# linnil1/KIR_graph

Measured on AMD Instinct MI355X. Metric: typed 150 bp PE reads/s (pileup+EM) per GPU; achieved HBM GB/s vs roofline, higher is better.
Workload: dtype f64

## Files before the change

include/graphkir_hip.h:

```cpp
#ifndef GRAPHKIR_HIP_H
#define GRAPHKIR_HIP_H

#include <stddef.h>
#include <stdint.h>

#ifdef __cplusplus
extern "C" {
#endif

#define GK_ABI_VERSION 1

#define GK_OK 0
#define GK_ERR_NO_DEVICE (-1)
#define GK_ERR_HIP (-2)
#define GK_ERR_ARG (-3)
#define GK_ERR_ASSERT (-4)
#define GK_ERR_CAPACITY (-5)

#define GK_MAX_CIG 14
#define GK_MAX_MM 16
#define GK_MAX_INS 6
#define GK_MAX_EVENTS 22
#define GK_CIG_M 0
#define GK_CIG_I 1
// ... 42 lines not shown
  uint8_t rsv1[16];
} gk_mate_wide;

typedef struct gk_ctx gk_ctx;
typedef struct gk_index gk_index;
typedef struct gk_tab gk_tab;
typedef struct gk_lut gk_lut;
typedef uint64_t gk_dptr;

int gk_abi_version(void);
const char* gk_last_error(void);
int gk_device_count(int* n);
int gk_ctx_create(int device, gk_ctx** out);
int gk_ctx_create_priority(int device, int urgent, gk_ctx** out);
int gk_ctx_destroy(gk_ctx* ctx);
int gk_sync(gk_ctx* ctx);
int gk_device_memory(gk_ctx* ctx, int64_t* free_bytes, int64_t* total_bytes, int64_t* pool_cached_bytes);
int gk_malloc(gk_ctx* ctx, size_t bytes, gk_dptr* out);
int gk_free(gk_ctx* ctx, gk_dptr p);
int gk_memset(gk_ctx* ctx, gk_dptr p, int value, size_t bytes);
int gk_h2d(gk_ctx* ctx, gk_dptr dst, const void* src, size_t bytes);
int gk_d2h(gk_ctx* ctx, void* dst, gk_dptr src, size_t bytes);
int gk_d2d(gk_ctx* ctx, gk_dptr dst, gk_dptr src, size_t bytes);
int gk_timer_start(gk_ctx* ctx);
int gk_timer_stop_ms(gk_ctx* ctx, float* ms);
int gk_prof_enable(gk_ctx* ctx, int on);
int gk_prof_kernel_count(void);
const char* gk_prof_kernel_name(int id);
int gk_prof_collect(gk_ctx* ctx, int64_t* launches, double* total_ms);

int gk_index_create(gk_ctx* ctx, const uint64_t* key, int32_t n_var, const int32_t* gene_vbeg,
                    int32_t n_gene, gk_index** out);
int gk_index_destroy(gk_index* idx);

typedef struct gk_tab_info {
  int64_t n_pairs;
  int64_t n_valid;
  int64_t n_ids;
  int32_t n_novel;
  int32_t err_flags;
  gk_dptr d_pair_src;
  gk_dptr d_off;
  gk_dptr d_ids;
  gk_dptr d_pair_gene;
  gk_dptr d_pair_nh;
  gk_dptr d_novel_key;
} gk_tab_info;
int gk_tabulate(gk_ctx* ctx, gk_index* idx, gk_dptr d_mates, int64_t n_pairs, gk_tab** out);
int gk_tabulate_corrected(gk_ctx* ctx, gk_index* idx, gk_dptr d_mates, int64_t n_pairs, gk_dptr d_corr,
                          gk_dptr d_gene_pos0, gk_tab** out);
int gk_tabulate_spilled(gk_ctx* ctx, gk_index* idx, gk_dptr d_mates, int64_t n_pairs, gk_dptr d_corr,
                        gk_dptr d_gene_pos0, const gk_mate_wide* wide, const int64_t* spill_pair, int64_t n_spill,
                        gk_tab** out);
int gk_tab_from_csr(gk_ctx* ctx, int32_t n_var_total, int64_t n_valid, const uint32_t* off, const uint32_t* ids,
                    const uint8_t* pair_gene, const uint8_t* pair_nh, gk_tab** out);
int gk_tab_get_info(gk_tab* tab, gk_tab_info* info);
int gk_tab_destroy(gk_tab* tab);

int gk_select_gene(gk_ctx* ctx, gk_tab* tab, int gene, int multiple, gk_dptr d_rows_out, int64_t* n_out);
int gk_select_nonempty(gk_ctx* ctx, gk_tab* tab, gk_dptr d_rows, int64_t n_rows, gk_dptr d_vflag,
                       gk_dptr d_rows_out, int64_t* n_out);

int gk_variant_count(gk_ctx* ctx, gk_tab* tab, gk_dptr d_rows, int64_t n_rows, gk_dptr d_vflag,
                     gk_dptr d_cnt);
int gk_variant_count_range(gk_ctx* ctx, gk_tab* tab, gk_dptr d_rows, int64_t n_rows, gk_dptr d_vflag,
                           gk_dptr d_cnt, int32_t vbeg, int32_t vend);
int gk_variant_correct(gk_ctx* ctx, gk_tab* tab, gk_dptr d_cnt, gk_dptr d_vflag);
int gk_variant_surviving(gk_ctx* ctx, gk_tab* tab, gk_dptr d_cnt, gk_dptr d_vflag, int64_t max_out,
                         int32_t* ord_out, uint32_t* pos_out, uint32_t* neg_out, int64_t* n_out);

int gk_variant_surviving_gene(gk_ctx* ctx, gk_tab* tab, gk_dptr d_cnt, gk_dptr d_vflag, int32_t gene, int32_t vbeg,
                              int32_t vend, int64_t max_out, int32_t* ord_out, uint32_t* pos_out, uint32_t* neg_out,
                              int64_t* n_out);
int gk_sample_prepare(gk_ctx* ctx, gk_tab* tab, int32_t multiple, gk_dptr d_vflag, gk_dptr d_cnt, gk_dptr d_rows,
                      int64_t* gene_off_out);
int gk_sample_prepare_all(gk_ctx* ctx, gk_tab* tab, int32_t multiple, gk_dptr d_vflag, gk_dptr d_cnt, gk_dptr d_rows,
                          int64_t* gene_off_out, int64_t max_out, int32_t* ord_out, uint32_t* pos_out, uint32_t* neg_out,
                          int64_t* n_out, uint64_t* novel_key_out);
int gk_sample_prepare_exon(gk_ctx* ctx, gk_tab* tab, int32_t multiple, gk_dptr d_vflag, gk_dptr d_cnt, gk_dptr d_rows,
                           int64_t* gene_off_out, int64_t max_out, int32_t* ord_out, uint32_t* pos_out, uint32_t* neg_out,
                           int64_t* n_out);

int gk_compat(gk_ctx* ctx, gk_tab* tab, gk_dptr d_rows, int64_t n_rows, gk_dptr d_vflag,
              int32_t vbeg, int32_t vend, gk_dptr d_mask, int32_t words, int32_t n_allele, int32_t keep_empty,
              gk_dptr d_probs, gk_dptr d_miss, gk_dptr d_nvar);

int gk_novel_assign(gk_ctx* ctx, gk_dptr d_probs, int64_t n_rows, int32_t n_cols, const uint32_t* col_entries,
                    int32_t n_entries, gk_dptr d_code, uint16_t* code_out, uint32_t* count_out, int32_t* first_out);
int gk_novel_confusion(gk_ctx* ctx, gk_tab* tab, gk_dptr d_rows, int64_t n_rows, gk_dptr d_code, gk_dptr d_vflag,
                       int32_t vbeg, int32_t vend, gk_dptr d_carry, const int32_t* entry_col, const int32_t* entry_slot,
                       int32_t n_entries, int32_t n_slots, uint64_t* totals_out, int64_t max_out, int32_t* slot_out,
                       int32_t* ord_out, uint32_t* count_out, uint64_t* key_out, int64_t* n_out);

int gk_lut_create(gk_ctx* ctx, int32_t log2_capacity, gk_lut** out);
int gk_lut_destroy(gk_lut* lut);
int gk_lut_collect(gk_lut* lut, gk_dptr d_vals, int64_t n);
int gk_lut_pending(gk_lut* lut, int32_t* n_total, int32_t* n_known);
int gk_lut_export(gk_lut* lut, int32_t first, int32_t count, double* keys_out);
int gk_lut_define(gk_lut* lut, int32_t first, int32_t count, const double* log_vals);
int gk_lut_apply(gk_lut* lut, gk_dptr d_in, gk_dptr d_out, int64_t n);
typedef int (*gk_log10_fn)(const double* values, int64_t n, double* out);
int gk_lut_resolve(gk_lut* lut, gk_log10_fn log10_fn, int32_t* n_new, int32_t* n_known, int32_t* n_undefined);
int gk_lut_resolve_stored(gk_lut* lut, gk_log10_fn log10_fn, int32_t* n_new, int32_t* n_known, int32_t* n_undefined);
int gk_lut_known(gk_lut* lut, int32_t* n_known);
int gk_compat_log(gk_ctx* ctx, gk_tab* tab, gk_dptr d_rows, int64_t n_rows, gk_dptr d_vflag,
                  int32_t vbeg, int32_t vend, gk_dptr d_mask, int32_t words, int32_t n_allele, int32_t keep_empty,
                  gk_lut* lut, gk_dptr d_log);

int gk_maxsum(gk_ctx* ctx, gk_dptr d_L, int64_t n_rows, int64_t ld, const int32_t* ids, int32_t n_sets,
              int32_t c_prev, const int32_t* cols, int32_t n_cols, double* out);
int gk_fraction(gk_ctx* ctx, gk_dptr d_L, int64_t n_rows, int64_t ld, const int32_t* ids,
                int32_t n_sets, int32_t c, double* frac_out);
int gk_setmax(gk_ctx* ctx, gk_dptr d_L, int64_t n_rows, int64_t ld, const int32_t* ids, int32_t n_sets,
              int32_t c, gk_dptr d_P);

int gk_compat_log_miss(gk_ctx* ctx, gk_tab* tab, gk_dptr d_rows, int64_t n_rows, gk_dptr d_vflag,
                       int32_t vbeg, int32_t vend, gk_dptr d_mask, int32_t words, int32_t n_allele,
                       int32_t keep_empty, gk_lut* lut, gk_dptr d_log, gk_dptr d_miss8, int64_t ldm, gk_dptr d_flags);
int gk_miss_colsum(gk_ctx* ctx, gk_dptr d_miss8, int64_t ldm, int32_t n_cols, gk_dptr d_msum);
int gk_compat_log_miss_cols(gk_ctx* ctx, gk_tab* tab, gk_dptr d_rows, int64_t n_rows, gk_dptr d_vflag,
                            int32_t vbeg, int32_t vend, gk_dptr d_mask, int32_t words, int32_t n_allele,
                            int32_t keep_empty, gk_lut* lut, const int32_t* table_cols, int32_t n_table_cols,
                            gk_dptr d_log, gk_dptr d_miss8, int64_t ldm, gk_dptr d_flags);
int gk_compat_log_miss_narrow(gk_ctx* ctx, gk_tab* tab, gk_dptr d_rows, int64_t n_rows, gk_dptr d_vflag,
                              int32_t vbeg, int32_t vend, gk_dptr d_mask, int32_t words, int32_t n_allele,
                              int32_t keep_empty, gk_lut* lut, const int32_t* table_cols, int32_t n_table_cols,
                              gk_dptr d_log, gk_dptr d_miss8, int64_t ldm, gk_dptr d_flags, gk_dptr d_msum);
int gk_compat_patch(gk_ctx* ctx, gk_lut* lut, gk_dptr d_log, int64_t n_rows, int32_t n_allele, gk_dptr d_miss8,
                    int64_t ldm, gk_dptr d_flags);
int gk_compat_index(gk_ctx* ctx, gk_tab* tab, gk_dptr d_rows, int64_t n_rows, gk_dptr d_vflag, int32_t vbeg,
                    int32_t vend, gk_dptr d_mask, int32_t words, int32_t n_allele, int32_t keep_empty, gk_lut* lut,
                    gk_dptr d_lidx, gk_dptr d_miss8, int64_t ldm, gk_dptr d_flags);
int gk_expand_index(gk_ctx* ctx, gk_lut* lut, gk_dptr d_lidx, int64_t ldi, int64_t n_rows, int32_t n_allele, gk_dptr d_L,
                    int64_t ld);
// ... 74 lines not shown
  int32_t n_allele;
  uint32_t stream;
} gk_boot_job;
int gk_em_bootstrap(gk_ctx* ctx, const gk_boot_job* jobs, int32_t n_jobs, int32_t n_boot, uint64_t seed,
                    int32_t iter_max, double diff_threshold,
                    double* prob_out,
                    int32_t* iters_out,
                    uint32_t* counts_out);

int gk_boot_row_counts(gk_ctx* ctx, int64_t n_rows, int32_t n_boot, int32_t boot_first, uint64_t seed, uint32_t stream,
                       gk_dptr d_W, int64_t ldw);
int gk_weighted_sums(gk_ctx* ctx, gk_dptr d_V, int64_t ld, int64_t n_rows, int32_t n_sets, gk_dptr d_W, int64_t ldw,
                     int32_t n_boot, double* out);

typedef struct gk_packer gk_packer;
int gk_packer_create(const char* const* gene_names, int32_t n_genes, const char* const* ins_strings,
                     int32_t n_ins, gk_packer** out);
int gk_packer_destroy(gk_packer* pk);
int gk_packer_feed(gk_packer* pk, const char* text, size_t n_bytes, int32_t final);
int gk_packer_counts(gk_packer* pk, int64_t* n_lines, int64_t* n_reads, int64_t* n_pairs, int64_t* n_strange,
                     int64_t* n_strings);
int gk_packer_error(gk_packer* pk, int32_t* kind, int64_t* line_index);
int gk_packer_set_output(gk_packer* pk, gk_mate* mates_out, int64_t capacity);
int gk_packer_records(gk_packer* pk, gk_mate* mates_out, int64_t* pair_lines_out);
int gk_packer_spilled(gk_packer* pk, int64_t* n_spilled_pairs);
int gk_packer_spill_records(gk_packer* pk, gk_mate_wide* wide_out, int64_t* pair_index_out);
const char* gk_packer_string(gk_packer* pk, int64_t i);

typedef struct gk_bam gk_bam;
int gk_bam_open(const char* path, int32_t name_sorted, gk_bam** out);
int gk_bam_close(gk_bam* bam);
int gk_bam_info(gk_bam* bam, int64_t* n_records, int64_t* header_bytes, int32_t* n_ref);
int gk_bam_header(gk_bam* bam, char* text_out, int64_t capacity);
int gk_bam_next(gk_bam* bam, char* text_out, int64_t capacity, int64_t* n_written);
int gk_bam_pack(gk_bam* bam, struct gk_packer* packer);
int gk_bam_write(const char* path, const char* sam_text, int64_t n_bytes, int32_t coordinate_sort);
int gk_bam_write_lines(const char* path, const char* header_text, int64_t n_header, const char* sam_text,
                       int64_t n_bytes, const int64_t* line_idx, int64_t n_lines, int32_t coordinate_sort);
int gk_json_write_reads(const char* path, const char* sam_text, int64_t n_bytes, const int64_t* pair_lines,
                        int64_t n_pairs, const int64_t* src, int64_t n_rows, const uint32_t* off,
                        const uint32_t* ids, const char* const* names, int64_t n_names,
                        const char* const* genes, int32_t n_genes, const uint8_t* gene_of, const uint8_t* nh);
int gk_bam_pileup(gk_bam* bam, const int64_t* gene_off, int32_t n_gene, uint32_t* counts_out);
int gk_bam_pileup_sites(const char* path, const int64_t* sites, int64_t n_sites, const uint64_t* name_keys,
                        const int32_t* key_group, int64_t n_keys, const int32_t* site_group, uint32_t* counts_out);
int gk_sam_name_keys(const char* sam_text, int64_t n_bytes, const int64_t* line_idx, int64_t n_lines, uint64_t* keys_out);
int gk_bam_write_lines_tagged(const char* path, const char* header_text, int64_t n_header, const char* rg_text,
                              int64_t n_rg, const char* sam_text, int64_t n_bytes, const int64_t* line_idx,
                              const int32_t* line_group, int64_t n_lines, const char* const* tags, int32_t n_tags,
                              int32_t coordinate_sort);

int gk_depth(gk_ctx* ctx, gk_tab* tab, gk_dptr d_mates, int32_t multiple, const int64_t* gene_off,
             int32_t n_gene, uint32_t* depth_out);

int gk_depth_write_tsv(const char* path, const char* const* genes, const int64_t* gene_off, int32_t n_genes,
                       const uint32_t* depth);

int gk_cn_fit(gk_ctx* ctx, const double* x, const double* density, int32_t bins, const double* bases,
              int32_t n_bases, const double* dev, int32_t n_cn, int32_t first_cn, double space,
              double* loglik_out);
int gk_cn_assign(gk_ctx* ctx, const double* x, int32_t bins, double base, const double* dev, int32_t n_cn,
                 int32_t first_cn, double space, int32_t* cn_of_bin_out);

typedef struct gk_comm gk_comm;
int gk_comm_unique_id(void* id_out, size_t capacity);
int gk_comm_create(gk_ctx* ctx, const void* id, size_t id_bytes, int32_t rank, int32_t world, gk_comm** out);
int gk_comm_destroy(gk_comm* comm);
int gk_allgather_f64(gk_comm* comm, const double* send, double* recv, int64_t n);
int gk_allreduce_max_f64(gk_comm* comm, double* inout, int64_t n);
int gk_comm_barrier(gk_comm* comm);

int gk_mates_compact(gk_ctx* ctx, gk_dptr d_mates, int64_t n_mates, gk_dptr* d_compact_out, int64_t* bytes_out);
int gk_mates_expand(gk_ctx* ctx, gk_dptr d_compact, int64_t n_mates, gk_dptr d_mates_out);
int gk_mates_compact_size(const gk_mate* mates, int64_t n_mates, int32_t n_threads, int64_t* n_words_out);
int gk_mates_compact_host(const gk_mate* mates, int64_t n_mates, int32_t n_threads, uint32_t* out, int64_t capacity_words);

int gk_host_alloc(size_t bytes, void** out);
int gk_host_free(void* p);
int gk_h2d_async(gk_ctx* ctx, gk_dptr dst, const void* src, size_t bytes);

#ifdef __cplusplus
}
#endif
#endif
```

kir_graph_amd/_lib.py:

```python
from __future__ import annotations

import ctypes as C
import threading
import os
from pathlib import Path

import numpy as np

LIB_NAME = "libgraphkir_hip.so"
_lib = None


class GkError(RuntimeError):
    """Error reported by the native library."""


class GkNoDevice(GkError):
    """No HIP device: the typing path cannot run (there is no CPU fallback)."""


_MM = np.dtype([("ref_off", "<u2"), ("base", "u1"), ("rsv", "u1")])
MATE_DTYPE = np.dtype([
    ("pos0", "<u4"), ("flag", "<u2"), ("ref", "u1"), ("nh", "u1"),
    ("nm", "u1"), ("n_cig", "u1"), ("n_mm", "u1"), ("n_ins", "u1"),
    ("cig", "<u2", (14,)), ("mm", _MM, (16,)), ("ins", "<u4", (6,)),
])
assert MATE_DTYPE.itemsize == 128

MATE_WIDE_DTYPE = np.dtype([
    ("pos0", "<u4"), ("flag", "<u2"), ("ref", "u1"), ("nh", "u1"), ("nm", "u1"), ("rsv0", "u1"),
    ("n_cig", "<u2"), ("n_mm", "<u2"), ("n_ins", "<u2"),
    ("cig", "<u4", (128,)), ("mm", "<u4", (256,)), ("ins", "<u4", (120,)), ("rsv1", "u1", (16,)),
])
assert MATE_WIDE_DTYPE.itemsize == 2048
SPILLED = 0xFF

CIG_M, CIG_I, CIG_D, CIG_S = 0, 1, 2, 4
NM_ABSENT = 255
MAX_CIG, MAX_MM, MAX_INS, MAX_EV = 14, 16, 6, 22


class GeneJob(C.Structure):
    _fields_ = [
        ("d_rows", C.c_uint64), ("n_rows", C.c_int64), ("d_mask", C.c_uint64), ("d_L", C.c_uint64),
        ("d_miss8", C.c_uint64), ("ldm", C.c_int64), ("d_msum", C.c_uint64), ("d_flags", C.c_uint64),
        ("d_lidx", C.c_uint64),
        ("vbeg", C.c_int32), ("vend", C.c_int32), ("words", C.c_int32), ("n_allele", C.c_int32),
        ("n_steps", C.c_int32), ("top_n", C.c_int32), ("bound_ok", C.c_int32), ("passes", C.c_int32),
        ("indexed", C.c_int32), ("patches", C.c_int32),
        ("table_of", C.c_int32), ("n_step_cols", C.c_int32), ("step_cols", C.c_void_p), ("step_cols_off", C.c_void_p),
        ("table_cols", C.c_void_p), ("n_table_cols", C.c_int32),
    ]


class EmJob(C.Structure):
    _fields_ = [
        ("d_rows", C.c_uint64), ("n_rows", C.c_int64), ("d_mask", C.c_uint64),
        ("vbeg", C.c_int32), ("vend", C.c_int32), ("words", C.c_int32), ("n_allele", C.c_int32),
        ("n_distinct", C.c_int32), ("iterations", C.c_int32),
    ]


class BootJob(C.Structure):
    _fields_ = [
        ("sets", C.c_void_p), ("count", C.c_void_p),
        ("n_sets", C.c_int32), ("words", C.c_int32), ("n_allele", C.c_int32), ("stream", C.c_uint32),
    ]


class TabInfo(C.Structure):
    _fields_ = [
        ("n_pairs", C.c_int64), ("n_valid", C.c_int64), ("n_ids", C.c_int64),
        ("n_novel", C.c_int32), ("err_flags", C.c_int32),
        ("d_pair_src", C.c_uint64), ("d_off", C.c_uint64), ("d_ids", C.c_uint64),
        ("d_pair_gene", C.c_uint64), ("d_pair_nh", C.c_uint64), ("d_novel_key", C.c_uint64),
    ]


def libPath() -> Path:
    return Path(__file__).resolve().parent / LIB_NAME


_SIGS = {
    "gk_abi_version": (C.c_int, []),
    "gk_last_error": (C.c_char_p, []),
    "gk_device_count": (C.c_int, [C.POINTER(C.c_int)]),
    "gk_ctx_create": (C.c_int, [C.c_int, C.POINTER(C.c_void_p)]),
    "gk_ctx_create_priority": (C.c_int, [C.c_int, C.c_int, C.POINTER(C.c_void_p)]),
    "gk_ctx_destroy": (C.c_int, [C.c_void_p]),
    "gk_sync": (C.c_int, [C.c_void_p]),
    "gk_device_memory": (C.c_int, [C.c_void_p, C.POINTER(C.c_int64), C.POINTER(C.c_int64), C.POINTER(C.c_int64)]),
    "gk_malloc": (C.c_int, [C.c_void_p, C.c_size_t, C.POINTER(C.c_uint64)]),
    "gk_free": (C.c_int, [C.c_void_p, C.c_uint64]),
    "gk_memset": (C.c_int, [C.c_void_p, C.c_uint64, C.c_int, C.c_size_t]),
    "gk_h2d": (C.c_int, [C.c_void_p, C.c_uint64, C.c_void_p, C.c_size_t]),
    "gk_d2h": (C.c_int, [C.c_void_p, C.c_void_p, C.c_uint64, C.c_size_t]),
    "gk_d2d": (C.c_int, [C.c_void_p, C.c_uint64, C.c_uint64, C.c_size_t]),
    "gk_timer_start": (C.c_int, [C.c_void_p]),
    "gk_timer_stop_ms": (C.c_int, [C.c_void_p, C.POINTER(C.c_float)]),
    "gk_prof_enable": (C.c_int, [C.c_void_p, C.c_int]),
    "gk_prof_kernel_count": (C.c_int, []),
    "gk_prof_kernel_name": (C.c_char_p, [C.c_int]),
    "gk_prof_collect": (C.c_int, [C.c_void_p, C.c_void_p, C.c_void_p]),
    "gk_index_create": (C.c_int, [C.c_void_p, C.c_void_p, C.c_int32, C.c_void_p, C.c_int32, C.POINTER(C.c_void_p)]),
    "gk_index_destroy": (C.c_int, [C.c_void_p]),
    "gk_tabulate": (C.c_int, [C.c_void_p, C.c_void_p, C.c_uint64, C.c_int64, C.POINTER(C.c_void_p)]),
    "gk_tabulate_spilled": (C.c_int, [C.c_void_p, C.c_void_p, C.c_uint64, C.c_int64, C.c_uint64, C.c_uint64,
                                     C.c_void_p, C.c_void_p, C.c_int64, C.POINTER(C.c_void_p)]),
    "gk_tabulate_corrected": (C.c_int, [C.c_void_p, C.c_void_p, C.c_uint64, C.c_int64, C.c_uint64, C.c_uint64,
                                        C.POINTER(C.c_void_p)]),
    "gk_tab_from_csr": (C.c_int, [C.c_void_p, C.c_int32, C.c_int64, C.c_void_p, C.c_void_p, C.c_void_p, C.c_void_p,
                                  C.POINTER(C.c_void_p)]),
    "gk_tab_get_info": (C.c_int, [C.c_void_p, C.POINTER(TabInfo)]),
    "gk_tab_destroy": (C.c_int, [C.c_void_p]),
    "gk_select_gene": (C.c_int, [C.c_void_p, C.c_void_p, C.c_int, C.c_int, C.c_uint64, C.POINTER(C.c_int64)]),
    "gk_select_nonempty": (C.c_int, [C.c_void_p, C.c_void_p, C.c_uint64, C.c_int64, C.c_uint64, C.c_uint64,
                                     C.POINTER(C.c_int64)]),
    "gk_variant_count": (C.c_int, [C.c_void_p, C.c_void_p, C.c_uint64, C.c_int64, C.c_uint64, C.c_uint64]),
    "gk_variant_count_range": (C.c_int, [C.c_void_p, C.c_void_p, C.c_uint64, C.c_int64, C.c_uint64, C.c_uint64,
                                         C.c_int32, C.c_int32]),
    "gk_variant_surviving": (C.c_int, [C.c_void_p, C.c_void_p, C.c_uint64, C.c_uint64, C.c_int64, C.c_void_p,
                                       C.c_void_p, C.c_void_p, C.POINTER(C.c_int64)]),
    "gk_variant_surviving_gene": (C.c_int, [C.c_void_p, C.c_void_p, C.c_uint64, C.c_uint64, C.c_int32, C.c_int32, C.c_int32,
                                            C.c_int64, C.c_void_p, C.c_void_p, C.c_void_p, C.POINTER(C.c_int64)]),
    "gk_sample_prepare": (C.c_int, [C.c_void_p, C.c_void_p, C.c_int32, C.c_uint64, C.c_uint64, C.c_uint64, C.c_void_p]),
    "gk_sample_prepare_all": (C.c_int, [C.c_void_p, C.c_void_p, C.c_int32, C.c_uint64, C.c_uint64, C.c_uint64, C.c_void_p,
                                       C.c_int64, C.c_void_p, C.c_void_p, C.c_void_p, C.POINTER(C.c_int64), C.c_void_p]),
    "gk_variant_correct": (C.c_int, [C.c_void_p, C.c_void_p, C.c_uint64, C.c_uint64]),
    "gk_compat": (C.c_int, [C.c_void_p, C.c_void_p, C.c_uint64, C.c_int64, C.c_uint64, C.c_int32, C.c_int32,
                            C.c_uint64, C.c_int32, C.c_int32, C.c_int32, C.c_uint64, C.c_uint64, C.c_uint64]),
    "gk_lut_create": (C.c_int, [C.c_void_p, C.c_int32, C.POINTER(C.c_void_p)]),
    "gk_lut_destroy": (C.c_int, [C.c_void_p]),
    "gk_lut_collect": (C.c_int, [C.c_void_p, C.c_uint64, C.c_int64]),
    "gk_lut_pending": (C.c_int, [C.c_void_p, C.POINTER(C.c_int32), C.POINTER(C.c_int32)]),
    "gk_lut_export": (C.c_int, [C.c_void_p, C.c_int32, C.c_int32, C.c_void_p]),
    "gk_lut_define": (C.c_int, [C.c_void_p, C.c_int32, C.c_int32, C.c_void_p]),
    "gk_lut_apply": (C.c_int, [C.c_void_p, C.c_uint64, C.c_uint64, C.c_int64]),
    "gk_bam_open": (C.c_int, [C.c_char_p, C.c_int32, C.POINTER(C.c_void_p)]),
    "gk_bam_close": (C.c_int, [C.c_void_p]),
    "gk_bam_info": (C.c_int, [C.c_void_p, C.POINTER(C.c_int64), C.POINTER(C.c_int64), C.POINTER(C.c_int32)]),
    "gk_bam_header": (C.c_int, [C.c_void_p, C.c_char_p, C.c_int64]),
    "gk_bam_pileup": (C.c_int, [C.c_void_p, C.c_void_p, C.c_int32, C.c_void_p]),
    "gk_bam_pileup_sites": (C.c_int, [C.c_char_p, C.c_void_p, C.c_int64, C.c_void_p, C.c_void_p, C.c_int64, C.c_void_p,
                                      C.c_void_p]),
    "gk_sam_name_keys": (C.c_int, [C.c_char_p, C.c_int64, C.c_void_p, C.c_int64, C.c_void_p]),
    "gk_bam_write_lines_tagged": (C.c_int, [C.c_char_p, C.c_char_p, C.c_int64, C.c_char_p, C.c_int64, C.c_char_p,
                                            C.c_int64, C.c_void_p, C.c_void_p, C.c_int64, C.c_void_p, C.c_int32,
                                            C.c_int32]),
    "gk_novel_assign": (C.c_int, [C.c_void_p, C.c_uint64, C.c_int64, C.c_int32, C.c_void_p, C.c_int32, C.c_uint64,
                                  C.c_void_p, C.c_void_p, C.c_void_p]),
    "gk_novel_confusion": (C.c_int, [C.c_void_p, C.c_void_p, C.c_uint64, C.c_int64, C.c_uint64, C.c_uint64, C.c_int32,
                                     C.c_int32, C.c_uint64, C.c_void_p, C.c_void_p, C.c_int32, C.c_int32, C.c_void_p,
                                     C.c_int64, C.c_void_p, C.c_void_p, C.c_void_p, C.c_void_p, C.POINTER(C.c_int64)]),
    "gk_bam_write": (C.c_int, [C.c_char_p, C.c_char_p, C.c_int64, C.c_int32]),
    "gk_bam_write_lines": (C.c_int, [C.c_char_p, C.c_char_p, C.c_int64, C.c_char_p, C.c_int64, C.c_void_p, C.c_int64,
                                     C.c_int32]),
    "gk_json_write_reads": (C.c_int, [C.c_char_p, C.c_char_p, C.c_int64, C.c_void_p, C.c_int64, C.c_void_p, C.c_int64,
                                      C.c_void_p, C.c_void_p, C.c_void_p, C.c_int64, C.c_void_p, C.c_int32,
                                      C.c_void_p, C.c_void_p]),
    "gk_bam_pack": (C.c_int, [C.c_void_p, C.c_void_p]),
    "gk_bam_next": (C.c_int, [C.c_void_p, C.c_void_p, C.c_int64, C.POINTER(C.c_int64)]),
    "gk_compat_log": (C.c_int, [C.c_void_p, C.c_void_p, C.c_uint64, C.c_int64, C.c_uint64, C.c_int32, C.c_int32,
                                C.c_uint64, C.c_int32, C.c_int32, C.c_int32, C.c_void_p, C.c_uint64]),
    "gk_maxsum": (C.c_int, [C.c_void_p, C.c_uint64, C.c_int64, C.c_int64, C.c_void_p, C.c_int32, C.c_int32,
                            C.c_void_p, C.c_int32, C.c_void_p]),
    "gk_fraction": (C.c_int, [C.c_void_p, C.c_uint64, C.c_int64, C.c_int64, C.c_void_p, C.c_int32, C.c_int32,
                              C.c_void_p]),
    "gk_setmax": (C.c_int, [C.c_void_p, C.c_uint64, C.c_int64, C.c_int64, C.c_void_p, C.c_int32, C.c_int32,
                            C.c_uint64]),
    "gk_packer_create": (C.c_int, [C.c_void_p, C.c_int32, C.c_void_p, C.c_int32, C.POINTER(C.c_void_p)]),
    "gk_packer_destroy": (C.c_int, [C.c_void_p]),
    "gk_packer_feed": (C.c_int, [C.c_void_p, C.c_char_p, C.c_size_t, C.c_int32]),
    "gk_packer_counts": (C.c_int, [C.c_void_p, C.POINTER(C.c_int64), C.POINTER(C.c_int64), C.POINTER(C.c_int64),
                                   C.POINTER(C.c_int64), C.POINTER(C.c_int64)]),
    "gk_packer_error": (C.c_int, [C.c_void_p, C.POINTER(C.c_int32), C.POINTER(C.c_int64)]),
    "gk_packer_records": (C.c_int, [C.c_void_p, C.c_void_p, C.c_void_p]),
    "gk_packer_set_output": (C.c_int, [C.c_void_p, C.c_void_p, C.c_int64]),
    "gk_packer_spilled": (C.c_int, [C.c_void_p, C.POINTER(C.c_int64)]),
    "gk_packer_spill_records": (C.c_int, [C.c_void_p, C.c_void_p, C.c_void_p]),
    "gk_packer_string": (C.c_char_p, [C.c_void_p, C.c_int64]),
    "gk_depth": (C.c_int, [C.c_void_p, C.c_void_p, C.c_uint64, C.c_int32, C.c_void_p, C.c_int32, C.c_void_p]),
    "gk_depth_write_tsv": (C.c_int, [C.c_char_p, C.c_void_p, C.c_void_p, C.c_int32, C.c_void_p]),
    "gk_cn_fit": (C.c_int, [C.c_void_p, C.c_void_p, C.c_void_p, C.c_int32, C.c_void_p, C.c_int32, C.c_void_p,
                            C.c_int32, C.c_int32, C.c_double, C.c_void_p]),
    "gk_cn_assign": (C.c_int, [C.c_void_p, C.c_void_p, C.c_int32, C.c_double, C.c_void_p, C.c_int32, C.c_int32,
                               C.c_double, C.c_void_p]),
    "gk_em_sets": (C.c_int, [C.c_void_p, C.c_void_p, C.c_uint64, C.c_int64, C.c_int32, C.c_int32, C.c_uint64,
                             C.c_int32, C.c_uint64]),
    "gk_em_distinct": (C.c_int, [C.c_void_p, C.c_uint64, C.c_int64, C.c_int32, C.c_int32, C.c_void_p, C.c_void_p,
                                 C.POINTER(C.c_int32)]),
    "gk_compat_log_miss_cols": (C.c_int, [C.c_void_p, C.c_void_p, C.c_uint64, C.c_int64, C.c_uint64, C.c_int32, C.c_int32,
                                          C.c_uint64, C.c_int32, C.c_int32, C.c_int32, C.c_void_p, C.c_void_p, C.c_int32,
                                          C.c_uint64, C.c_uint64, C.c_int64, C.c_uint64]),
    "gk_compat_log_miss_narrow": (C.c_int, [C.c_void_p, C.c_void_p, C.c_uint64, C.c_int64, C.c_uint64, C.c_int32, C.c_int32,
                                            C.c_uint64, C.c_int32, C.c_int32, C.c_int32, C.c_void_p, C.c_void_p, C.c_int32,
                                            C.c_uint64, C.c_uint64, C.c_int64, C.c_uint64, C.c_uint64]),
    "gk_compat_log_miss": (C.c_int, [C.c_void_p, C.c_void_p, C.c_uint64, C.c_int64, C.c_uint64, C.c_int32, C.c_int32,
                                     C.c_uint64, C.c_int32, C.c_int32, C.c_int32, C.c_void_p, C.c_uint64, C.c_uint64,
                                     C.c_int64, C.c_uint64]),
    "gk_miss_colsum": (C.c_int, [C.c_void_p, C.c_uint64, C.c_int64, C.c_int32, C.c_uint64]),
    "gk_compat_index": (C.c_int, [C.c_void_p, C.c_void_p, C.c_uint64, C.c_int64, C.c_uint64, C.c_int32, C.c_int32,
                                  C.c_uint64, C.c_int32, C.c_int32, C.c_int32, C.c_void_p, C.c_uint64, C.c_uint64,
                                  C.c_int64, C.c_uint64]),
    "gk_expand_index": (C.c_int, [C.c_void_p, C.c_void_p, C.c_uint64, C.c_int64, C.c_int64, C.c_int32, C.c_uint64,
                                  C.c_int64]),
    "gk_bound_step": (C.c_int, [C.c_void_p, C.c_uint64, C.c_int64, C.c_int64, C.c_uint64, C.c_void_p, C.c_int32,
                                C.c_int32, C.c_void_p, C.c_int32, C.c_void_p, C.c_int32, C.c_int32, C.c_void_p,
                                C.c_void_p, C.c_void_p]),
    "gk_setsum": (C.c_int, [C.c_void_p, C.c_uint64, C.c_int64, C.c_int64, C.c_void_p, C.c_int32, C.c_int32,
                            C.c_void_p, C.c_void_p]),
    "gk_search_run": (C.c_int, [C.c_void_p, C.c_uint64, C.c_int64, C.c_int64, C.c_int32, C.c_uint64, C.c_int64,
                                C.c_uint64, C.c_void_p, C.c_int32, C.c_int32, C.c_int32, C.c_void_p, C.c_void_p,
                                C.POINTER(C.c_void_p)]),
    "gk_sample_search": (C.c_int, [C.c_void_p, C.c_void_p, C.c_int32, C.c_void_p, C.c_uint64, C.c_void_p, C.c_void_p,
                                   C.c_int32, C.c_void_p, C.c_void_p, C.c_void_p]),
    "gk_lut_resolve": (C.c_int, [C.c_void_p, C.c_void_p, C.POINTER(C.c_int32), C.POINTER(C.c_int32),
                                 C.POINTER(C.c_int32)]),
    "gk_sample_prepare_exon": (C.c_int, [C.c_void_p, C.c_void_p, C.c_int32, C.c_uint64, C.c_uint64, C.c_uint64, C.c_void_p,
                                         C.c_int64, C.c_void_p, C.c_void_p, C.c_void_p, C.POINTER(C.c_int64)]),
    "gk_sample_em": (C.c_int, [C.c_void_p, C.c_void_p, C.c_void_p, C.c_int32, C.c_int32, C.c_double, C.c_void_p, C.c_void_p]),
    "gk_mates_compact": (C.c_int, [C.c_void_p, C.c_uint64, C.c_int64, C.POINTER(C.c_uint64), C.POINTER(C.c_int64)]),
    "gk_mates_expand": (C.c_int, [C.c_void_p, C.c_uint64, C.c_int64, C.c_uint64]),
    "gk_mates_compact_size": (C.c_int, [C.c_void_p, C.c_int64, C.c_int32, C.POINTER(C.c_int64)]),
    "gk_mates_compact_host": (C.c_int, [C.c_void_p, C.c_int64, C.c_int32, C.c_void_p, C.c_int64]),
    "gk_compat_patch": (C.c_int, [C.c_void_p, C.c_void_p, C.c_uint64, C.c_int64, C.c_int32, C.c_uint64, C.c_int64, C.c_uint64]),
    "gk_lut_resolve_stored": (C.c_int, [C.c_void_p, C.c_void_p, C.POINTER(C.c_int32), C.POINTER(C.c_int32),
                                        C.POINTER(C.c_int32)]),
    "gk_lut_known": (C.c_int, [C.c_void_p, C.POINTER(C.c_int32)]),
    "gk_search_steps": (C.c_int, [C.c_void_p, C.POINTER(C.c_int32)]),
    "gk_search_info": (C.c_int, [C.c_void_p, C.c_int32, C.POINTER(C.c_int32), C.POINTER(C.c_int64),
                                 C.POINTER(C.c_int32)]),
    "gk_search_copy": (C.c_int, [C.c_void_p, C.c_int32, C.c_void_p, C.c_void_p, C.c_void_p, C.c_void_p]),
    "gk_search_export": (C.c_int, [C.c_void_p, C.c_int32, C.c_void_p, C.c_void_p, C.c_void_p, C.c_void_p, C.c_void_p, C.c_void_p]),
    "gk_search_colsum": (C.c_int, [C.c_void_p, C.c_void_p]),
    "gk_search_log": (C.c_int, [C.c_void_p, C.c_void_p, C.c_int64, C.POINTER(C.c_int64)]),
    "gk_search_destroy": (C.c_int, [C.c_void_p]),
    "gk_site_verdict_tallies": (C.c_int, [C.c_void_p, C.c_int64, C.c_void_p, C.c_int64, C.c_void_p, C.c_void_p, C.c_void_p,
                                         C.c_int64, C.c_int32, C.POINTER(C.c_int32)]),
    "gk_site_verdict_genes": (C.c_int, [C.c_void_p, C.c_int64, C.c_void_p, C.c_int64, C.c_void_p, C.c_void_p, C.c_void_p,
                                       C.c_void_p, C.c_int32, C.c_void_p, C.c_void_p]),
    "gk_site_verdict": (C.c_int, [C.c_void_p, C.c_void_p, C.c_void_p, C.c_void_p, C.c_int64, C.c_int32,
                                  C.POINTER(C.c_int32)]),
    "gk_comm_unique_id": (C.c_int, [C.c_void_p, C.c_size_t]),
    "gk_comm_create": (C.c_int, [C.c_void_p, C.c_void_p, C.c_size_t, C.c_int32, C.c_int32, C.POINTER(C.c_void_p)]),
    "gk_comm_destroy": (C.c_int, [C.c_void_p]),
    "gk_allgather_f64": (C.c_int, [C.c_void_p, C.c_void_p, C.c_void_p, C.c_int64]),
    "gk_allreduce_max_f64": (C.c_int, [C.c_void_p, C.c_void_p, C.c_int64]),
    "gk_comm_barrier": (C.c_int, [C.c_void_p]),
    "gk_host_alloc": (C.c_int, [C.c_size_t, C.POINTER(C.c_void_p)]),
    "gk_host_free": (C.c_int, [C.c_void_p]),
    "gk_h2d_async": (C.c_int, [C.c_void_p, C.c_uint64, C.c_void_p, C.c_size_t]),
    "gk_em_run": (C.c_int, [C.c_void_p, C.c_void_p, C.c_void_p, C.c_int32, C.c_int32, C.c_int32, C.c_int32,
                            C.c_double, C.c_void_p, C.POINTER(C.c_int32)]),
    "gk_em_bootstrap": (C.c_int, [C.c_void_p, C.c_void_p, C.c_int32, C.c_int32, C.c_uint64, C.c_int32, C.c_double,
                                  C.c_void_p, C.c_void_p, C.c_void_p]),
    "gk_boot_row_counts": (C.c_int, [C.c_void_p, C.c_int64, C.c_int32, C.c_int32, C.c_uint64, C.c_uint32, C.c_uint64,
                                     C.c_int64]),
    "gk_weighted_sums": (C.c_int, [C.c_void_p, C.c_uint64, C.c_int64, C.c_int64, C.c_int32, C.c_uint64, C.c_int64, C.c_int32,
                                   C.c_void_p]),
}

EXPORTED = sorted(_SIGS)

ARGSORT_FN = C.CFUNCTYPE(C.c_int, C.POINTER(C.c_double), C.c_int64, C.POINTER(C.c_int64))


def _numpy_argsort(values, n, order_out):
    try:
        v = np.ctypeslib.as_array(values, shape=(n,))
        np.ctypeslib.as_array(order_out, shape=(n,))[:] = np.argsort(v)
        return 0
    except Exception:
# ... 249 lines not shown
```

kir_graph_amd/cohort.py:

```python
from __future__ import annotations

import os

import numpy as np


def prefetched(items, prepare, depth: int = 1, workers: int = 1):
    from concurrent.futures import ThreadPoolExecutor
    items = iter(items)
    with ThreadPoolExecutor(max_workers=max(1, workers), thread_name_prefix="gk-prefetch") as pool:
        pending = []
        for item in items:
            pending.append(pool.submit(prepare, item))
            if len(pending) > depth:
                yield pending.pop(0).result()
        while pending:
            yield pending.pop(0).result()


def overlapped(items, work, lanes: int = 2):
    from concurrent.futures import ThreadPoolExecutor
    import queue
    if lanes <= 1:
        for item in items:
# ... 29 lines not shown
        quota, period = open("/sys/fs/cgroup/cpu.max").read().split()[:2]
        if quota != "max":
            cores = min(cores, max(1, int(quota) // int(period)))
    except (OSError, ValueError):
        pass
    private = os.environ.get("GK_PRIVATE_CORES") == "1"
    ranks = 1 if private else max(1, int(os.environ.get("LOCAL_WORLD_SIZE") or os.environ.get("WORLD_SIZE") or 1))
    return max(1, cores // ranks)


def pipelineDefaults(procs: int = 1, cores: int | None = None) -> None:
    cores = hostCoresPerRank() if cores is None else cores
    lanes, slots = (5, 3) if cores >= 6 else (4, 2) if cores >= 3 else (3, 2)
    os.environ.setdefault("GK_WAIT_POLICY", "block")
    os.environ.setdefault("GK_SAMPLE_LANES", str(lanes))
    os.environ.setdefault("GK_SEARCH_SLOTS", str(slots))


def sampleLanes() -> int:
    return max(1, int(os.environ.get("GK_SAMPLE_LANES", "3")))


def stagingContexts(dev, lanes: int | None = None):
    lanes = sampleLanes() if lanes is None else lanes
    base = lanes
    ingest = dev.worker(base, urgent=True)
    return dev.worker(base + 1), ingest


def stagedSamples(items, copy_in, tabulate, depth: int | None = None):
    depth = int(os.environ.get("GK_PREFETCH", "1")) if depth is None else depth
    if depth <= 0:
        for item in items:
            yield tabulate(item if copy_in is None else copy_in(item))
        return
    if copy_in is None:
        yield from prefetched(items, tabulate, depth=depth)
    else:
        yield from prefetched(prefetched(items, copy_in, depth=depth), tabulate, depth=depth)


def sampleFootprint(data, method: str) -> int:
    tab = getattr(data, "tab", None)
    if tab is None:
        return 0
    tables = getattr(data.index, "tables", None) or []
    mean_alleles = sum(t.n_allele for t in tables) / max(len(tables), 1)
    n = int(tab.n_valid)
    if method in ("em", "report"):
        per_read = 4.0 * (mean_alleles / 32 + 1) + 16
    else:
        per_read = 9.2 * mean_alleles * (2 if method.startswith(("exonfirst", "pv_exonfirst")) else 1)
    lists = 4.0 * int(tab.n_ids) + 48.0 * n
    records = 256.0 * int(tab.n_pairs) if getattr(tab, "mates", None) is not None else 0.0
    return int(1.15 * per_read * n + lists + records)


def hbmBudget(dev=None) -> int:
    env = os.environ.get("GK_HBM_BUDGET_GB")
    if env:
        return int(float(env) * (1 << 30))
    try:
        if dev is None:
            from .kir_typing import defaultDevice
            dev = defaultDevice()
        return int(0.55 * dev.memory()[1])
    except Exception:
        return 0


class SampleTyper:

    def __init__(self, method: str, lanes: int | None = None, top_n: int = 600, variant_correction: bool = True,
                 finish=None, **typer_kwargs):
        from concurrent.futures import ThreadPoolExecutor
        import queue
        self.method = "exonfirst_1" if method == "exonfirst" else method
        self.lanes = sampleLanes() if lanes is None else max(1, lanes)
        self.top_n, self.variant_correction = top_n, variant_correction
        self.finish = finish
        self.typer_kwargs = typer_kwargs
        self._pool = ThreadPoolExecutor(max_workers=self.lanes, thread_name_prefix="gk-sample") if self.lanes > 1 else None
        self._free = queue.SimpleQueue()
        for lane in range(self.lanes):
            self._free.put(lane)
        self._pending: list = []
        import threading
        self._room = threading.Condition()
        self._inflight_bytes, self._budget = 0, None

    def _admit(self, data) -> int:
        need = sampleFootprint(data, self.method)
        if need <= 0 or self._pool is None:
            return 0
        if self._budget is None:
            self._budget = hbmBudget(getattr(getattr(data, "tab", None), "dev", None))
        if self._budget <= 0:
            return 0
        with self._room:
            while self._inflight_bytes > 0 and self._inflight_bytes + need > self._budget:
                self._room.wait(timeout=1.0)
            self._inflight_bytes += need
        return need

    def _release(self, need: int) -> None:
        if need:
            with self._room:
                self._inflight_bytes -= need
                self._room.notify_all()

    def typeOne(self, data, gene_cn, item=None, lane: int = 0):
        from .kir_typing import selectKirTypingModel
        typer = selectKirTypingModel(self.method, data, top_n=self.top_n, variant_correction=self.variant_correction,
                                     **self.typer_kwargs)
        typer.slot_base = lane
        calls, warnings = typer.typing(gene_cn() if callable(gene_cn) else gene_cn)
        if self.finish is not None:
            return self.finish(typer, calls, warnings, item)
        return calls, warnings, typer

    def _run(self, data, gene_cn, item, need: int = 0):
        lane = self._free.get()
        try:
            return self.typeOne(data, gene_cn, item, lane)
        finally:
            self._free.put(lane)
            self._release(need)

    def submit(self, data, gene_cn, item=None) -> None:
        if self._pool is None:
            self._pending.append(_Done(self.typeOne(data, gene_cn, item, 0)))
        else:
            self._pending.append(self._pool.submit(self._run, data, gene_cn, item, self._admit(data)))

    def inFlight(self) -> int:
        return len(self._pending)

    def next(self):
        return self._pending.pop(0).result()

    def drain(self):
        while self._pending:
            yield self.next()

    def close(self) -> None:
        if self._pool is not None:
            self._pool.shutdown(wait=True)
            self._pool = None

    def __enter__(self):
        return self

    def __exit__(self, *exc):
        self.close()


class _Done:
    def __init__(self, value):
        self._value = value

    def result(self):
        return self._value


def typeSamples(samples, method: str, lanes: int | None = None, finish=None, top_n: int = 600,
                variant_correction: bool = True):
    with SampleTyper(method, lanes=lanes, top_n=top_n, variant_correction=variant_correction, finish=finish) as typer:
        for data, gene_cn, item in samples:
            typer.submit(data, gene_cn, item)
            if typer.inFlight() >= typer.lanes:
                yield typer.next()
        yield from typer.drain()


def shardSamples(n_samples: int, world: int, weights=None) -> list[list[int]]:
    if weights is None:
        return [list(range(r, n_samples, world)) for r in range(world)]
    assert len(weights) == n_samples
    load = [0.0] * world
    shards: list[list[int]] = [[] for _ in range(world)]
    for i in sorted(range(n_samples), key=lambda i: (-float(weights[i]), i)):
        r = min(range(world), key=lambda r: (load[r], len(shards[r]), r))
        shards[r].append(i)
        load[r] += float(weights[i])
    return [sorted(s) for s in shards]


def sampleWeights(paths: list) -> list[float] | None:
    out = []
    for group in paths:
        total = 0
        for p in ([group] if isinstance(group, str) else group):
            if not p:
                continue
            try:
                total += os.path.getsize(p)
            except OSError:
                return None
        out.append(float(total))
    return out if any(out) else None

# ... 52 lines not shown
```

kir_graph_amd/csrc/gk_depth.hip:

```cpp
#include "gk_common.h"

namespace {

constexpr int kThreads = 256;

__global__ __launch_bounds__(kThreads) void depth_mark(const gk_mate* __restrict__ mates,
                                                       const gk_mate_wide* __restrict__ wide,
                                                       const int32_t* __restrict__ pair_src,
                                                       const uint8_t* __restrict__ pair_nh, int64_t n_valid,
                                                       int multiple, const int64_t* __restrict__ gene_off, int n_gene,
                                                       uint32_t* __restrict__ diff) {
  const int64_t t = (int64_t)blockIdx.x * kThreads + threadIdx.x;
  if (t >= 2 * n_valid) return;
  const int64_t i = t >> 1;
  if (!multiple && pair_nh[i] != 1) return;
  const gk_mate& m = mates[2 * (int64_t)pair_src[i] + (t & 1)];
  if (m.ref >= n_gene) return;
  const int64_t base = gene_off[m.ref], len = gene_off[m.ref + 1] - base;
  int64_t cur = m.pos0;
  auto run = [&](uint32_t op, uint32_t n) {
    if (op == GK_CIG_M) {
      const int64_t a = cur < 0 ? 0 : cur, b = cur + n > len ? len : cur + n;
      if (b > a) {
        atomicAdd(&diff[base + a], 1u);
        atomicAdd(&diff[base + b], 0xFFFFFFFFu);
      }
      cur += n;
    } else if (op == GK_CIG_D) {
      cur += n;
    }
  };
  if (m.n_cig == GK_SPILLED) {
    if (!wide) return;
    const gk_mate_wide& x = wide[2 * (int64_t)m.ins[0] + (t & 1)];
    const int n_cig = x.n_cig < GK_WIDE_CIG ? x.n_cig : GK_WIDE_CIG;
    for (int c = 0; c < n_cig; ++c) run(x.cig[c] & 15u, x.cig[c] >> 4);
    return;
  }
  const int n_cig = m.n_cig < GK_MAX_CIG ? m.n_cig : GK_MAX_CIG;
  for (int c = 0; c < n_cig; ++c) run(m.cig[c] & 15u, m.cig[c] >> 4);
}

__global__ __launch_bounds__(kThreads) void depth_finish(const uint32_t* excl, const uint32_t* diff, int64_t n,
                                                         uint32_t* depth ) {
  const int64_t i = (int64_t)blockIdx.x * kThreads + threadIdx.x;
  if (i < n) depth[i] = excl[i] + diff[i];
}

}

extern "C" int gk_depth(gk_ctx* ctx, gk_tab* tab, gk_dptr d_mates, int32_t multiple, const int64_t* gene_off,
                        int32_t n_gene, uint32_t* depth_out) {
  gk_bind(ctx);
  GK_REQUIRE(ctx && tab && gene_off && depth_out && n_gene > 0, "bad depth arguments");
  GK_REQUIRE(tab->d_pair_src, "depth needs a tabulation made from packed records");
  const int64_t total = gene_off[n_gene];
  hipStream_t st = ctx->stream;
  uint32_t *diff = nullptr, *scan = nullptr;
  int64_t* d_off = nullptr;
  GK_HIP(gk_pool_malloc(ctx, (void**)&diff, (size_t)(total + 1) * sizeof(uint32_t)));
  GK_HIP(gk_pool_malloc(ctx, (void**)&scan, (size_t)(total + 1) * sizeof(uint32_t)));
  GK_HIP(gk_pool_malloc(ctx, (void**)&d_off, (size_t)(n_gene + 1) * sizeof(int64_t)));
  GK_HIP(hipMemsetAsync(diff, 0, (size_t)(total + 1) * sizeof(uint32_t), st));
  GK_HIP(hipMemcpyAsync(d_off, gene_off, (size_t)(n_gene + 1) * sizeof(int64_t), hipMemcpyHostToDevice, st));
  if (tab->n_valid)
    GK_KERNEL(depth_mark, dim3((unsigned)((2 * tab->n_valid + kThreads - 1) / kThreads)), dim3(kThreads), 0, st,
                       gk_ptr<const gk_mate>(d_mates), tab->d_wide, tab->d_pair_src, tab->d_pair_nh, tab->n_valid, multiple, d_off,
                       n_gene, diff);
  GK_HIP(hipMemcpyAsync(scan, diff, (size_t)(total + 1) * sizeof(uint32_t), hipMemcpyDeviceToDevice, st));
  int rc = gk_scan_u32(ctx, scan, total + 1, nullptr);
  if (rc) return rc;
  GK_KERNEL(depth_finish, dim3((unsigned)((total + kThreads - 1) / kThreads)), dim3(kThreads), 0, st, scan, diff,
                     total, diff);
  GK_HIP(hipGetLastError());
  GK_HIP(hipMemcpyAsync(depth_out, diff, (size_t)total * sizeof(uint32_t), hipMemcpyDeviceToHost, st));
  GK_HIP(hipStreamSynchronize(st));
  gk_pool_free(ctx, diff);
  gk_pool_free(ctx, scan);
  gk_pool_free(ctx, d_off);
  return GK_OK;
}
```

kir_graph_amd/csrc/gk_tabulate.hip:

```cpp
#include <algorithm>
#include <vector>

#include "gk_common.h"

namespace {

constexpr int kThreads = 256;
constexpr int kMaxEv = GK_MAX_EVENTS;
constexpr uint64_t kEmpty = ~0ull;

constexpr int kMateWords = sizeof(gk_mate) / 4;
constexpr int kCigWord = 3;
constexpr int kMmWord = kCigWord + GK_MAX_CIG / 2;
constexpr int kInsWord = kMmWord + GK_MAX_MM;
static_assert(sizeof(gk_mate) == 128 && kInsWord + GK_MAX_INS == kMateWords, "gk_mate layout");
constexpr int kRecLd = kMateWords + 1;
constexpr int kEvLd = kMaxEv + 1;
constexpr int kMaskWords = 8;

constexpr uint32_t kEvNovel = 1u << 31;
constexpr uint32_t kEvIsN = 1u << 30;
constexpr uint32_t kEvOrdMask = (1u << 26) - 1;
constexpr uint32_t kEvSlotMask = (1u << 30) - 1;

struct MateView {
  static constexpr int kCapCig = GK_MAX_CIG, kCapMm = GK_MAX_MM, kCapIns = GK_MAX_INS, kCapEv = kMaxEv;
  const uint32_t* w;
  __device__ bool spilled() const { return n_cig() == GK_SPILLED; }
  __device__ uint32_t pos0() const { return w[0]; }
  __device__ uint32_t flag() const { return w[1] & 0xFFFFu; }
  __device__ uint32_t ref() const { return (w[1] >> 16) & 0xFFu; }
  __device__ uint32_t nm() const { return w[2] & 0xFFu; }
  __device__ uint32_t n_cig() const { return (w[2] >> 8) & 0xFFu; }
  __device__ uint32_t n_mm() const { return (w[2] >> 16) & 0xFFu; }
  __device__ uint32_t cig(int i) const {
    const uint32_t word = w[kCigWord + (i >> 1)];
    return (i & 1) ? (word >> 16) : (word & 0xFFFFu);
  }
  __device__ uint32_t mm_off(int i) const { return w[kMmWord + i] & 0xFFFFu; }
  __device__ uint32_t mm_base(int i) const { return (w[kMmWord + i] >> 16) & 0xFFu; }
  __device__ uint32_t ins(int i) const { return w[kInsWord + i]; }
  __device__ bool passes() const { return (flag() & 2u) && nm() != GK_NM_ABSENT && nm() <= 4u; }
};

constexpr int kHeadWords = 16;
constexpr int kHeadLd = kHeadWords + 1;
struct HeadView {
  static constexpr int kCapCig = GK_MAX_CIG, kCapMm = GK_MAX_MM, kCapIns = GK_MAX_INS, kCapEv = kMaxEv;
  const uint32_t* w;
  const uint32_t* g;
  __device__ uint32_t word(int i) const { return i < kHeadWords ? w[i] : g[i]; }
  __device__ bool spilled() const { return n_cig() == GK_SPILLED; }
  __device__ uint32_t pos0() const { return w[0]; }
  __device__ uint32_t flag() const { return w[1] & 0xFFFFu; }
  __device__ uint32_t ref() const { return (w[1] >> 16) & 0xFFu; }
  __device__ uint32_t nm() const { return w[2] & 0xFFu; }
  __device__ uint32_t n_cig() const { return (w[2] >> 8) & 0xFFu; }
  __device__ uint32_t n_mm() const { return (w[2] >> 16) & 0xFFu; }
  __device__ uint32_t cig(int i) const {
    const uint32_t x = w[kCigWord + (i >> 1)];
    return (i & 1) ? (x >> 16) : (x & 0xFFFFu);
  }
  __device__ uint32_t mm_off(int i) const { return word(kMmWord + i) & 0xFFFFu; }
  __device__ uint32_t mm_base(int i) const { return (word(kMmWord + i) >> 16) & 0xFFu; }
  __device__ uint32_t ins(int i) const { return g[kInsWord + i]; }
  __device__ bool passes() const { return (flag() & 2u) && nm() != GK_NM_ABSENT && nm() <= 4u; }
};
static_assert(kCigWord + GK_MAX_CIG / 2 <= kHeadWords, "the CIGAR lies in the staged head");

struct WideView {
  static constexpr int kCapCig = GK_WIDE_CIG, kCapMm = GK_WIDE_MM, kCapIns = GK_WIDE_INS, kCapEv = GK_WIDE_EVENTS;
  const gk_mate_wide* p;
  __device__ uint32_t pos0() const { return p->pos0; }
  __device__ uint32_t flag() const { return p->flag; }
  __device__ uint32_t ref() const { return p->ref; }
  __device__ uint32_t nm() const { return p->nm; }
  __device__ uint32_t n_cig() const { return p->n_cig; }
  __device__ uint32_t n_mm() const { return p->n_mm; }
  __device__ uint32_t cig(int i) const { return p->cig[i]; }
  __device__ uint32_t mm_off(int i) const { return p->mm[i] >> 8; }
  __device__ uint32_t mm_base(int i) const { return p->mm[i] & 0xFFu; }
  __device__ uint32_t ins(int i) const { return p->ins[i]; }
  __device__ bool passes() const { return (flag() & 2u) && nm() != GK_NM_ABSENT && nm() <= 4u; }
};
static_assert(sizeof(gk_mate_wide) == 2048, "gk_mate_wide layout");

__device__ inline void stage_heads(const gk_mate* mates, int64_t m0, int64_t n_mates, uint32_t* rec) {
  const int n_rec = (int)min<int64_t>(kThreads, n_mates - m0);
#pragma unroll
  for (int k = 0; k < kHeadWords / 4; ++k) {
    const int idx = threadIdx.x + kThreads * k;
    const int rcd = idx >> 2, part = idx & 3;
    if (rcd < n_rec) {
      const uint4 v = reinterpret_cast<const uint4*>(mates + m0 + rcd)[part];
      uint32_t* d = rec + rcd * kHeadLd + part * 4;
      d[0] = v.x; d[1] = v.y; d[2] = v.z; d[3] = v.w;
    }
  }
  __syncthreads();
}

__device__ inline void stage_mates(const gk_mate* mates, int64_t m0, int64_t n_mates, uint32_t* rec) {
  const uint4* src = reinterpret_cast<const uint4*>(mates + m0);
  const int n_vec = (int)min<int64_t>(kThreads, n_mates - m0) * (kMateWords / 4);
#pragma unroll
  for (int k = 0; k < kMateWords / 4; ++k) {
    const int idx = threadIdx.x + kThreads * k;
    if (idx < n_vec) {
      const uint4 v = src[idx];
      uint32_t* d = rec + (idx >> 3) * kRecLd + (idx & 7) * 4;
      d[0] = v.x; d[1] = v.y; d[2] = v.z; d[3] = v.w;
    }
  }
  __syncthreads();
}

struct IndexView {
  const uint64_t* key;
  const int32_t* bucket;
  const int32_t* gene_boff;
  int n_var, n_gene;
// ... 282 lines not shown
                                            uint32_t* more ) {
  auto keep_word = [&](uint32_t w, uint32_t word) {
    if (w == 0) first[0] = word; else if (w == 1) first[1] = word; else if (w == 2) first[2] = word;
    else if (w == 3) first[3] = word; else more[w - kMaskRegs] = word;
  };
  if (len == 0) return 0;
  if (any_n || len > 32u * kMaskWords) {
    uint32_t kept = 0, cur = 0;
    for (uint32_t c = 0; c < len; ++c) {
      const uint32_t i = lo + c;
      if (negative_kept(ix.key[i], (int)i, ix, ev, n_ev, any_n, right)) {
        ++kept;
        cur |= 1u << (c & 31u);
      }
      if ((c & 31u) == 31u || c + 1 == len) {
        if (c < 32u * kMaskWords) keep_word(c >> 5, cur);
        cur = 0;
      }
    }
    return kept;
  }
  uint32_t rel4[4];
#pragma unroll
  for (int q = 0; q < 4; ++q) rel4[q] = q < n_ev ? (ev.r[q] & ~kEvIsN) - lo : 0xFFFFFFFFu;
  const uint32_t n_words = (len + 31u) >> 5;
  uint32_t kept = 0;
  for (uint32_t w = 0; w < n_words; ++w) {
    const uint32_t left = len - 32u * w;
    uint32_t word = left >= 32u ? ~0u : ((1u << left) - 1u);
#pragma unroll
    for (int q = 0; q < 4; ++q) {
      const uint32_t rel = rel4[q] - 32u * w;
      if (rel < 32u) word &= ~(1u << rel);
    }
    for (int e = 4; e < n_ev; ++e) {
      const uint32_t rel = (ev.more[e - kEvRegs] & ~kEvIsN) - lo - 32u * w;
      if (rel < 32u) word &= ~(1u << rel);
    }
    const uint32_t first = lo + 32u * w, sh = first & 31u;
    const uint32_t a = ix.del_bits[first >> 5], b = ix.del_bits[(first >> 5) + 1];
    uint32_t dels = (sh ? (a >> sh) | (b << (32u - sh)) : a) & word;
    while (dels) {
      const int bit = __ffs(dels) - 1;
      dels &= dels - 1;
      const uint64_t k = ix.key[first + (uint32_t)bit];
      if (gk_key_pos(k) + gk_key_val(k) + 10u >= right) word &= ~(1u << bit);
    }
    kept += (uint32_t)__popc(word);
    keep_word(w, word);
  }
  return kept;
}

__global__ __launch_bounds__(kThreads) void tab_count(const gk_mate* mates, int64_t n_mates, IndexView ix,
                                                      NovelTable nt, uint32_t* cnt ,
                                                      uint32_t* valid , int* err_flags,
                                                      uint4* ev_save ,
                                                      uint32_t* ev_more ,
                                                      uint32_t* lo_save ,
                                                      uint4* mask_save ,
                                                      uint32_t* mask_more ) {
  __shared__ uint32_t rec[kThreads * kHeadLd];
  const int64_t m0 = (int64_t)blockIdx.x * kThreads;
  stage_heads(mates, m0, n_mates, rec);
  const int64_t m = m0 + threadIdx.x;
  const bool in = m < n_mates;
  const HeadView r{rec + threadIdx.x * kHeadLd, reinterpret_cast<const uint32_t*>(mates + (in ? m : 0))};
  EvRow ev{{0u, 0u, 0u, 0u}, ev_more + (in ? m : 0) * kEvMore, nt.keys};
  const bool ok = in && r.passes() && !r.spilled();
  const bool ok_other = __shfl_xor((int)ok, 1, 64) != 0;
  const bool pair_ok = ok && ok_other;
  const int64_t pair = m >> 1;
  const int side = (int)(m & 1);
  uint32_t n_pos = 0;
  Walked wk;
  wk.n = 0; wk.lo = wk.hi = 0; wk.right = 0; wk.any_n = 0;
  bool enumerate = false;
  if (pair_ok) {
    walk_mate<false>(r, ix, nt, m, ev, nullptr, 0, 0, wk);
    if (wk.overflow) atomicOr(err_flags, 2);
    if (wk.clipped) {
    } else if (wk.bad_window) {
      atomicOr(err_flags, 1);
    } else if (!wk.drop) {
      n_pos = wk.n;
      enumerate = true;
    }
  }
  uint32_t kept_bits[kMaskRegs] = {0u, 0u, 0u, 0u};
  const uint32_t n_neg = enumerate ? window_negatives(ix, ev, wk.n, wk.any_n, wk.right, (uint32_t)wk.lo,
                                                      (uint32_t)(wk.hi - wk.lo), kept_bits,
                                                      mask_more + (in ? m : 0) * (kMaskWords - kMaskRegs))
                                   : 0u;
  if (!in) return;
  cnt[4 * pair + side] = n_pos;
  cnt[4 * pair + 2 + side] = n_neg;
  if (side == 0) valid[pair] = pair_ok ? 1u : 0u;
  if (enumerate && (uint32_t)(wk.hi - wk.lo) > 32u * kMaskWords)
    atomicOr(err_flags, 4);
  ev_save[m] = make_uint4(ev.r[0], ev.r[1], ev.r[2], ev.r[3]);
  mask_save[m] = make_uint4(kept_bits[0], kept_bits[1], kept_bits[2], kept_bits[3]);
  lo_save[m] = (uint32_t)wk.lo;
}

constexpr int kExpandThreads = 128;
constexpr int kExpandWaves = kExpandThreads / 64;
constexpr uint32_t kExpandCap = 4096;

__global__ __launch_bounds__(kExpandThreads) void tab_expand(int64_t n_mates, int n_var, const uint32_t* rank,
                                                             const uint32_t* off, const uint32_t* valid,
                                                             const uint4* ev_save, const uint32_t* ev_more,
                                                             const uint32_t* lo_save, const uint4* mask_save,
                                                             const uint32_t* mask_more, uint32_t* ids) {
  __shared__ uint32_t stage[kExpandWaves][kExpandCap];
  const int lane = threadIdx.x & 63;
  const int wid = __builtin_amdgcn_readfirstlane(threadIdx.x >> 6);
  const int64_t m0 = ((int64_t)blockIdx.x * kExpandWaves + wid) * 64;
  if (m0 >= n_mates) return;
  const int64_t m = m0 + lane;
  const int64_t pair0 = m0 >> 1, pair_end = min<int64_t>((m0 + 64) >> 1, n_mates >> 1);
// ... 138 lines not shown
                                                     IndexView ix, NovelTable nt, uint32_t* cnt,
                                                     uint32_t* valid, int* err_flags, uint32_t* evw_all) {
  const int64_t t = (int64_t)blockIdx.x * 64 + threadIdx.x;
  const bool in = t < 2 * n_spill;
  const WideView r{wide + (in ? t : 0)};
  const bool ok = in && r.passes();
  const bool ok_other = __shfl_xor((int)ok, 1, 64) != 0;
  const bool pair_ok = ok && ok_other;
  if (!in) return;
  const int64_t pair = spill_pair[t >> 1];
  const int side = (int)(t & 1);
  uint32_t* evw = evw_all + t * GK_WIDE_EVENTS;
  uint32_t n_pos = 0, n_neg = 0;
  if (pair_ok) {
    Walked wk;
    EvPtr ev{evw, nullptr};
    walk_mate<false>(r, ix, nt, 2 * pair + side, ev, nullptr, 0, 0, wk);
    if (wk.overflow) atomicOr(err_flags, 2);
    if (wk.clipped) {
    } else if (wk.bad_window) {
      atomicOr(err_flags, 1);
    } else if (!wk.drop) {
      n_pos = (uint32_t)wk.n;
      for (int i = wk.lo; i < wk.hi; ++i)
        n_neg += negative_kept(ix.key[i], i, ix, EvView{evw}, wk.n, wk.any_n, wk.right) ? 1u : 0u;
    }
  }
  cnt[4 * pair + side] = n_pos;
  cnt[4 * pair + 2 + side] = n_neg;
  if (side == 0) valid[pair] = pair_ok ? 2u : 0u;
}

__global__ __launch_bounds__(64) void tab_emit_wide(const gk_mate_wide* wide, const int64_t* spill_pair, int64_t n_spill,
                                                    IndexView ix, NovelTable nt, const uint32_t* off,
                                                    const uint32_t* valid, uint32_t* ids, uint32_t* evw_all) {
  const int64_t t = (int64_t)blockIdx.x * 64 + threadIdx.x;
  if (t >= 2 * n_spill) return;
  const int64_t pair = spill_pair[t >> 1];
  const int side = (int)(t & 1);
  if (!valid[pair]) return;
  const uint32_t o_pos = off[4 * pair + side], o_pos_end = off[4 * pair + side + 1];
  const uint32_t o_neg = off[4 * pair + 2 + side], o_neg_end = off[4 * pair + 2 + side + 1];
  if (o_pos == o_pos_end && o_neg == o_neg_end) return;
  const WideView r{wide + t};
  uint32_t* evw = evw_all + t * GK_WIDE_EVENTS;
  Walked wk;
  EvPtr ev{evw, nullptr};
  walk_mate<true>(r, ix, nt, 2 * pair + side, ev, ids, o_pos, o_pos_end, wk);
  uint32_t at = o_neg;
  for (int i = wk.lo; i < wk.hi && at < o_neg_end; ++i)
    if (negative_kept(ix.key[i], i, ix, EvView{evw}, wk.n, wk.any_n, wk.right)) ids[at++] = (uint32_t)i;
}

__global__ __launch_bounds__(kThreads) void gather_pairs(const gk_mate* mates, const int32_t* pair_src, int64_t n_valid,
                                                         const uint32_t* off_in, uint32_t* off_out, uint8_t* gene,
                                                         uint8_t* nh, uint32_t total) {
  const int64_t i = (int64_t)blockIdx.x * kThreads + threadIdx.x;
  if (i > n_valid) return;
  if (i == n_valid) {
    off_out[4 * n_valid] = total;
    return;
  }
  const int64_t p = pair_src[i];
#pragma unroll
  for (int k = 0; k < 4; ++k) off_out[4 * i + k] = off_in[4 * p + k];
  const uint32_t w1 = reinterpret_cast<const uint32_t*>(mates + 2 * p)[1];
  gene[i] = (uint8_t)((w1 >> 16) & 0xFFu);
  nh[i] = (uint8_t)(w1 >> 24);
}

__device__ inline int mate_used_words(const uint32_t* w, int* n_cw, int* n_mm, int* n_ins) {
  const uint32_t h = w[2];
  const int n_cig = (int)((h >> 8) & 0xFFu);
  const bool spilled = n_cig == GK_SPILLED;
  *n_cw = spilled ? 0 : (min(n_cig, GK_MAX_CIG) + 1) / 2;
  *n_mm = spilled ? 0 : min((int)((h >> 16) & 0xFFu), GK_MAX_MM);
  *n_ins = spilled ? 1 : min((int)(h >> 24), GK_MAX_INS);
  return 3 + *n_cw + *n_mm + *n_ins;
}

__global__ __launch_bounds__(kThreads) void mates_count_words(const gk_mate* mates, int64_t n, uint32_t* cnt) {
  const int64_t m = (int64_t)blockIdx.x * kThreads + threadIdx.x;
  if (m >= n) return;
  int a, b, c;
  cnt[m] = (uint32_t)mate_used_words(reinterpret_cast<const uint32_t*>(mates + m), &a, &b, &c);
}

__global__ __launch_bounds__(kThreads) void mates_pack_words(const gk_mate* mates, int64_t n, const uint32_t* off,
                                                             uint32_t* off_out, uint32_t* words, uint32_t total) {
  const int64_t m = (int64_t)blockIdx.x * kThreads + threadIdx.x;
  if (m > n) return;
  if (m == n) { off_out[n] = total; return; }
  const uint32_t* w = reinterpret_cast<const uint32_t*>(mates + m);
  int n_cw, n_mm, n_ins;
  mate_used_words(w, &n_cw, &n_mm, &n_ins);
  uint32_t* d = words + off[m];
  off_out[m] = off[m];
  d[0] = w[0]; d[1] = w[1]; d[2] = w[2];
  d += 3;
  for (int i = 0; i < n_cw; ++i) d[i] = w[kCigWord + i];
  d += n_cw;
  for (int i = 0; i < n_mm; ++i) d[i] = w[kMmWord + i];
  d += n_mm;
  for (int i = 0; i < n_ins; ++i) d[i] = w[kInsWord + i];
}

__global__ __launch_bounds__(kThreads) void mates_unpack_words(const uint32_t* off, const uint32_t* words, int64_t n,
                                                               gk_mate* mates) {
  const int64_t m = (int64_t)blockIdx.x * kThreads + threadIdx.x;
  if (m >= n) return;
  const uint32_t* s = words + off[m];
  uint32_t rec[kMateWords];
#pragma unroll
  for (int i = 0; i < kMateWords; ++i) rec[i] = 0u;
  rec[0] = s[0]; rec[1] = s[1]; rec[2] = s[2];
  int n_cw, n_mm, n_ins;
  mate_used_words(rec, &n_cw, &n_mm, &n_ins);
  uint32_t* d = reinterpret_cast<uint32_t*>(mates + m);
  uint4* d4 = reinterpret_cast<uint4*>(d);
// ... 62 lines not shown
        for (int32_t v = ia; v < v1 && key[v] <= kb; ++v)
          if (key[v] == kb) at = v;
        snp_ord.push_back(at);
      }
    }
    lb_a.push_back(v1);
    lb_t.push_back(v1);
    for (int q = 0; q < 4; ++q) snp_ord.push_back(-1);
  }
  GK_HIP(gk_pool_malloc(ctx, (void**)&idx->d_snp_ord, snp_ord.size() * sizeof(int32_t)));
  GK_HIP(hipMemcpyAsync(idx->d_snp_ord, snp_ord.data(), snp_ord.size() * sizeof(int32_t), hipMemcpyHostToDevice, ctx->stream));
  GK_HIP(gk_pool_malloc(ctx, (void**)&idx->d_lb_a, lb_a.size() * sizeof(int32_t)));
  GK_HIP(gk_pool_malloc(ctx, (void**)&idx->d_lb_t, lb_t.size() * sizeof(int32_t)));
  GK_HIP(gk_pool_malloc(ctx, (void**)&idx->d_gene_pbase, pbase.size() * sizeof(int32_t)));
  GK_HIP(hipMemcpyAsync(idx->d_lb_a, lb_a.data(), lb_a.size() * sizeof(int32_t), hipMemcpyHostToDevice, ctx->stream));
  GK_HIP(hipMemcpyAsync(idx->d_lb_t, lb_t.data(), lb_t.size() * sizeof(int32_t), hipMemcpyHostToDevice, ctx->stream));
  GK_HIP(hipMemcpyAsync(idx->d_gene_pbase, pbase.data(), pbase.size() * sizeof(int32_t), hipMemcpyHostToDevice, ctx->stream));
  std::vector<uint32_t> del_bits((size_t)(n_var + 31) / 32 + 2, 0u);
  for (int32_t v = 0; v < n_var; ++v)
    if (gk_key_typ(key[v]) == GK_TYP_DEL) del_bits[(size_t)v >> 5] |= 1u << (v & 31);
  GK_HIP(gk_pool_malloc(ctx, (void**)&idx->d_del_bits, del_bits.size() * sizeof(uint32_t)));
  GK_HIP(hipMemcpyAsync(idx->d_del_bits, del_bits.data(), del_bits.size() * sizeof(uint32_t), hipMemcpyHostToDevice, ctx->stream));
  GK_HIP(hipStreamSynchronize(ctx->stream));
  *out = idx;
  return GK_OK;
}

int gk_index_destroy(gk_index* idx) {
  gk_bind(idx ? idx->ctx : nullptr);
  if (!idx) return GK_OK;
  gk_ctx* ctx = idx->ctx;
  gk_pool_free(ctx,idx->d_key);
  gk_pool_free(ctx,idx->d_gene_vbeg);
  gk_pool_free(ctx,idx->d_bucket);
  gk_pool_free(ctx,idx->d_gene_boff);
  gk_pool_free(ctx,idx->d_del_bits);
  gk_pool_free(ctx,idx->d_lb_a);
  gk_pool_free(ctx,idx->d_lb_t);
  gk_pool_free(ctx,idx->d_gene_pbase);
  gk_pool_free(ctx,idx->d_snp_ord);
  delete idx;
  return GK_OK;
}

int gk_tabulate(gk_ctx* ctx, gk_index* idx, gk_dptr d_mates_p, int64_t n_pairs, gk_tab** out) {
  return gk_tabulate_corrected(ctx, idx, d_mates_p, n_pairs, 0, 0, out);
}

int gk_tabulate_corrected(gk_ctx* ctx, gk_index* idx, gk_dptr d_mates_p, int64_t n_pairs, gk_dptr d_corr,
                          gk_dptr d_gene_pos0, gk_tab** out) {
  return gk_tabulate_spilled(ctx, idx, d_mates_p, n_pairs, d_corr, d_gene_pos0, nullptr, nullptr, 0, out);
}

static int tabulate_with_table(gk_ctx* ctx, gk_index* idx, gk_dptr d_mates_p, int64_t n_pairs, gk_dptr d_corr,
                               gk_dptr d_gene_pos0, const gk_mate_wide* wide, const int64_t* spill_pair,
                               int64_t n_spill, uint32_t log2cap, bool* table_too_small, gk_tab** out);

int gk_tabulate_spilled(gk_ctx* ctx, gk_index* idx, gk_dptr d_mates_p, int64_t n_pairs, gk_dptr d_corr,
                        gk_dptr d_gene_pos0, const gk_mate_wide* wide, const int64_t* spill_pair, int64_t n_spill,
                        gk_tab** out) {
  uint32_t log2cap = 16;
  while ((1ull << log2cap) < (uint64_t)(2 * std::max<int64_t>(n_pairs, 0)) && log2cap < 22) ++log2cap;
  log2cap = (uint32_t)std::min<long>(30, std::max<long>(4, gk_test_hook_value("novel_log2cap", (long)log2cap)));
  uint32_t log2max = 16;
  while ((1ull << log2max) < (uint64_t)(2 * std::max<int64_t>(n_pairs, 0)) * GK_WIDE_EVENTS * 2 && log2max < 30) ++log2max;
  for (;;) {
    bool too_small = false;
    const int rc = tabulate_with_table(ctx, idx, d_mates_p, n_pairs, d_corr, d_gene_pos0, wide, spill_pair, n_spill, log2cap,
                                       &too_small, out);
    if (!too_small) return rc;
    if (log2cap >= log2max) return rc;
    log2cap = std::min(log2cap + 3, log2max);
  }
}

static int tabulate_with_table(gk_ctx* ctx, gk_index* idx, gk_dptr d_mates_p, int64_t n_pairs, gk_dptr d_corr,
                               gk_dptr d_gene_pos0, const gk_mate_wide* wide, const int64_t* spill_pair,
                               int64_t n_spill, uint32_t log2cap, bool* table_too_small, gk_tab** out) {
  gk_bind(ctx);
  GK_REQUIRE(ctx && idx && out && n_pairs >= 0, "bad tabulate arguments");
  GK_REQUIRE(n_spill >= 0 && n_spill <= n_pairs && (n_spill == 0 || (wide && spill_pair)), "bad wide-pair arguments");
  for (int64_t k = 0; k < n_spill; ++k)
    GK_REQUIRE(spill_pair[k] >= 0 && spill_pair[k] < n_pairs && (k == 0 || spill_pair[k - 1] < spill_pair[k]),
               "wide pairs must name pairs of the sample, ascending");
  GK_REQUIRE((d_corr == 0) == (d_gene_pos0 == 0), "correction table and position offsets come together");
  GK_REQUIRE(n_pairs < (1ll << 26), "more than 2^26 pairs per call");
  const gk_mate* mates = gk_ptr<const gk_mate>(d_mates_p);
  const int64_t n_mates = 2 * n_pairs;
  hipStream_t st = ctx->stream;
  gk_tab* tab = new gk_tab();
  tab->ctx = ctx; tab->idx = idx; tab->n_pairs = n_pairs; tab->n_var = idx->n_var;

  NovelTable nt;
  const size_t cap = 1ull << log2cap;
  nt.mask = (uint32_t)(cap - 1);
  GK_HIP(gk_pool_malloc(ctx, (void**)&nt.keys, cap * sizeof(uint64_t)));
  GK_HIP(gk_pool_malloc(ctx, (void**)&nt.seq, cap * sizeof(uint64_t)));
  GK_HIP(gk_pool_malloc(ctx, (void**)&nt.rank, cap * sizeof(uint32_t)));
  GK_HIP(hipMemsetAsync(nt.keys, 0xFF, cap * sizeof(uint64_t), st));
  GK_HIP(hipMemsetAsync(nt.seq, 0xFF, cap * sizeof(uint64_t), st));

  uint32_t *cnt = nullptr, *valid = nullptr, *lo_save = nullptr, *ev_more = nullptr, *mask_more = nullptr;
  uint4 *ev_save = nullptr, *mask_save = nullptr;
  int* d_err = nullptr;
  GK_HIP(gk_pool_malloc(ctx, (void**)&ev_save, (size_t)(n_mates + 1) * sizeof(uint4)));
  GK_HIP(gk_pool_malloc(ctx, (void**)&ev_more, (size_t)(n_mates + 1) * kEvMore * sizeof(uint32_t)));
  GK_HIP(gk_pool_malloc(ctx, (void**)&lo_save, (size_t)(n_mates + 1) * sizeof(uint32_t)));
  GK_HIP(gk_pool_malloc(ctx, (void**)&mask_save, (size_t)(n_mates + 1) * sizeof(uint4)));
  GK_HIP(gk_pool_malloc(ctx, (void**)&mask_more, (size_t)(n_mates + 1) * (kMaskWords - kMaskRegs) * sizeof(uint32_t)));
  GK_HIP(gk_pool_malloc(ctx, (void**)&cnt, (size_t)(4 * n_pairs + 2) * sizeof(uint32_t)));
  GK_HIP(gk_pool_malloc(ctx, (void**)&valid, (size_t)(n_pairs + 1) * sizeof(uint32_t)));
  GK_HIP(gk_pool_malloc(ctx, (void**)&d_err, sizeof(int)));
  GK_HIP(hipMemsetAsync(d_err, 0, sizeof(int), st));
  nt.flags = d_err;

  const IndexView ix{idx->d_key, idx->d_bucket, idx->d_gene_boff, idx->n_var, idx->n_gene,
                     gk_ptr<uint8_t>(d_corr), gk_ptr<int64_t>(d_gene_pos0), idx->d_del_bits, idx->d_lb_a, idx->d_lb_t,
                     idx->d_gene_pbase, idx->d_snp_ord};
  if (n_mates) {
    GK_PROF(ctx, "tab_count", GK_KERNEL(tab_count, dim3(nblk(n_mates)), dim3(kThreads), 0, st, mates, n_mates, ix,
                       nt, cnt, valid, d_err, ev_save, ev_more, lo_save, mask_save, mask_more));
  }
  int64_t* d_spill_pair = nullptr;
  uint32_t* wide_ev = nullptr;
  if (n_spill) {
    GK_HIP(gk_pool_malloc(ctx, (void**)&tab->d_wide, (size_t)(2 * n_spill) * sizeof(gk_mate_wide)));
    GK_HIP(gk_pool_malloc(ctx, (void**)&d_spill_pair, (size_t)n_spill * sizeof(int64_t)));
    GK_HIP(gk_pool_malloc(ctx, (void**)&wide_ev, (size_t)(2 * n_spill) * GK_WIDE_EVENTS * sizeof(uint32_t)));
    GK_HIP(hipMemcpyAsync(tab->d_wide, wide, (size_t)(2 * n_spill) * sizeof(gk_mate_wide), hipMemcpyHostToDevice, st));
    GK_HIP(hipMemcpyAsync(d_spill_pair, spill_pair, (size_t)n_spill * sizeof(int64_t), hipMemcpyHostToDevice, st));
    GK_HIP(hipStreamSynchronize(st));
    tab->n_spill = n_spill;
    GK_KERNEL(tab_count_wide, dim3(nblk(2 * n_spill, 64)), dim3(64), 0, st, tab->d_wide, d_spill_pair, n_spill, ix, nt,
              cnt, valid, d_err, wide_ev);
  }
  int rc = gk_scan_u32(ctx, cnt, 4 * n_pairs, cnt + 4 * n_pairs);
  if (rc) return rc;

  const int64_t n_words = n_mates + 1;
  uint32_t *bitmap = nullptr, *prefix = nullptr, *wide_bits = nullptr;
  GK_HIP(gk_pool_malloc(ctx, (void**)&bitmap, (size_t)n_words * sizeof(uint32_t)));
  GK_HIP(gk_pool_malloc(ctx, (void**)&prefix, (size_t)(n_words + 1) * sizeof(uint32_t)));
  GK_HIP(gk_pool_malloc(ctx, (void**)&wide_bits, (size_t)(2 * n_spill + 1) * kWideWords * sizeof(uint32_t)));
  GK_HIP(hipMemsetAsync(bitmap, 0, (size_t)n_words * sizeof(uint32_t), st));
  GK_HIP(hipMemsetAsync(wide_bits, 0, (size_t)(2 * n_spill + 1) * kWideWords * sizeof(uint32_t), st));
  GK_PROF(ctx, "novel_mark", GK_KERNEL(novel_mark, dim3(nblk((int64_t)cap)), dim3(kThreads), 0, st, nt, bitmap, wide_bits,
                                     d_spill_pair, n_spill));
  GK_PROF(ctx, "novel_count", GK_KERNEL(novel_count, dim3(nblk(n_words)), dim3(kThreads), 0, st, bitmap, prefix, n_words));
  if (n_spill)
    GK_KERNEL(novel_count_wide, dim3(nblk(2 * n_spill)), dim3(kThreads), 0, st, wide_bits, d_spill_pair, n_spill, prefix);
  rc = gk_scan_u32(ctx, prefix, n_words, prefix + n_words);
  if (rc) return rc;

  uint32_t totals[2] = {0, 0};
  int err = 0;
  GK_HIP(gk_fetch_queue(ctx, &totals[0], cnt + 4 * n_pairs, sizeof(uint32_t)));
  GK_HIP(gk_fetch_queue(ctx, &totals[1], prefix + n_words, sizeof(uint32_t)));
  GK_HIP(gk_fetch_queue(ctx, &err, d_err, sizeof(int)));
  GK_HIP(gk_fetch_wait(ctx));
  tab->n_ids = totals[0];
  tab->n_novel = (int32_t)totals[1];
  tab->err_flags = err & 3;
  if ((err & 8) || (uint64_t)tab->n_novel * 2 > cap) {
    gk_set_error("novel variant table overflow (%d novel variants in %llu slots)", tab->n_novel, (unsigned long long)cap);
    *table_too_small = true;
    GK_HIP(hipStreamSynchronize(st));
    gk_pool_free(ctx,cnt); gk_pool_free(ctx,valid); gk_pool_free(ctx,d_err); gk_pool_free(ctx,bitmap); gk_pool_free(ctx,prefix); gk_pool_free(ctx,wide_bits);
    gk_pool_free(ctx,ev_save); gk_pool_free(ctx,lo_save); gk_pool_free(ctx,mask_save); gk_pool_free(ctx,ev_more); gk_pool_free(ctx,mask_more);
    gk_pool_free(ctx,d_spill_pair); gk_pool_free(ctx,wide_ev);
    gk_pool_free(ctx,nt.keys); gk_pool_free(ctx,nt.seq); gk_pool_free(ctx,nt.rank);
    gk_tab_destroy(tab);
    return GK_ERR_CAPACITY;
  }

  GK_HIP(gk_pool_malloc(ctx, (void**)&tab->d_novel_key, (size_t)(tab->n_novel + 1) * sizeof(uint64_t)));
  GK_PROF(ctx, "novel_assign", GK_KERNEL(novel_assign, dim3(nblk((int64_t)cap)), dim3(kThreads), 0, st, nt, bitmap, wide_bits,
                     d_spill_pair, n_spill, prefix, tab->d_novel_key));

  GK_HIP(gk_pool_malloc(ctx, (void**)&tab->d_ids, (size_t)(tab->n_ids + 1) * sizeof(uint32_t)));
  if (n_mates) {
    const bool two_walks = gk_test_hook("two_walks");
    if ((err & 4) || two_walks) {
      GK_PROF(ctx, "tab_emit", GK_KERNEL(tab_emit, dim3(nblk(n_mates)), dim3(kThreads), 0, st, mates, n_mates, ix, nt,
                         cnt, valid, tab->d_ids));
    } else {
      GK_PROF(ctx, "tab_expand", GK_KERNEL(tab_expand, dim3(nblk(n_mates, kExpandThreads)), dim3(kExpandThreads), 0, st, n_mates, idx->n_var,
                         nt.rank, cnt, valid, ev_save, ev_more, lo_save, mask_save, mask_more, tab->d_ids));
    }
    if (n_spill)
      GK_KERNEL(tab_emit_wide, dim3(nblk(2 * n_spill, 64)), dim3(64), 0, st, tab->d_wide, d_spill_pair, n_spill, ix, nt,
                cnt, valid, tab->d_ids, wide_ev);
  }
  GK_HIP(gk_pool_malloc(ctx, (void**)&tab->d_pair_src, (size_t)(n_pairs + 1) * sizeof(int32_t)));
  rc = gk_compact(ctx, valid, nullptr, n_pairs, tab->d_pair_src, &tab->n_valid);
  if (rc) return rc;
  GK_HIP(gk_pool_malloc(ctx, (void**)&tab->d_off, (size_t)(4 * tab->n_valid + 1) * sizeof(uint32_t)));
  GK_HIP(gk_pool_malloc(ctx, (void**)&tab->d_pair_gene, (size_t)tab->n_valid + 1));
  GK_HIP(gk_pool_malloc(ctx, (void**)&tab->d_pair_nh, (size_t)tab->n_valid + 1));
  GK_PROF(ctx, "gather_pairs", GK_KERNEL(gather_pairs, dim3(nblk(tab->n_valid + 1)), dim3(kThreads), 0, st, mates, tab->d_pair_src,
                     tab->n_valid, cnt, tab->d_off, tab->d_pair_gene, tab->d_pair_nh, (uint32_t)tab->n_ids));
  GK_HIP(hipGetLastError());
  GK_HIP(hipStreamSynchronize(st));
  gk_pool_free(ctx,cnt); gk_pool_free(ctx,valid); gk_pool_free(ctx,d_err); gk_pool_free(ctx,bitmap); gk_pool_free(ctx,prefix); gk_pool_free(ctx,wide_bits);
  gk_pool_free(ctx,ev_save); gk_pool_free(ctx,lo_save); gk_pool_free(ctx,mask_save); gk_pool_free(ctx,ev_more); gk_pool_free(ctx,mask_more);
  gk_pool_free(ctx,d_spill_pair); gk_pool_free(ctx,wide_ev);
  gk_pool_free(ctx,nt.keys); gk_pool_free(ctx,nt.seq); gk_pool_free(ctx,nt.rank);
  if (err & 2) {
    gk_set_error("a filter-passing mate carries more variant events than its record format allows (%d, wide %d)", kMaxEv,
                 GK_WIDE_EVENTS);
    gk_tab_destroy(tab);
    return GK_ERR_CAPACITY;
  }
  *out = tab;
  return GK_OK;
}

int gk_tab_from_csr(gk_ctx* ctx, int32_t n_var_total, int64_t n_valid, const uint32_t* off, const uint32_t* ids,
                    const uint8_t* pair_gene, const uint8_t* pair_nh, gk_tab** out) {
  gk_bind(ctx);
  GK_REQUIRE(ctx && out && off && pair_gene && pair_nh && n_valid >= 0 && n_var_total >= 0, "bad CSR arguments");
  const int64_t n_ids = off[4 * n_valid];
  for (int64_t i = 0; i < 4 * n_valid; ++i) GK_REQUIRE(off[i] <= off[i + 1], "CSR offsets must be non-decreasing");
  for (int64_t i = 0; i < n_ids; ++i) GK_REQUIRE(ids[i] < (uint32_t)n_var_total, "variant ordinal out of range");
  gk_tab* tab = new gk_tab();
  tab->ctx = ctx; tab->n_pairs = n_valid; tab->n_valid = n_valid; tab->n_ids = n_ids;
  tab->n_var = n_var_total; tab->n_novel = 0;
  hipStream_t st = ctx->stream;
  GK_HIP(gk_pool_malloc(ctx, (void**)&tab->d_off, (size_t)(4 * n_valid + 1) * sizeof(uint32_t)));
  GK_HIP(gk_pool_malloc(ctx, (void**)&tab->d_ids, (size_t)(n_ids + 1) * sizeof(uint32_t)));
  GK_HIP(gk_pool_malloc(ctx, (void**)&tab->d_pair_gene, (size_t)n_valid + 1));
  GK_HIP(gk_pool_malloc(ctx, (void**)&tab->d_pair_nh, (size_t)n_valid + 1));
  GK_HIP(hipMemcpyAsync(tab->d_off, off, (size_t)(4 * n_valid + 1) * sizeof(uint32_t), hipMemcpyHostToDevice, st));
  if (n_ids) GK_HIP(hipMemcpyAsync(tab->d_ids, ids, (size_t)n_ids * sizeof(uint32_t), hipMemcpyHostToDevice, st));
  if (n_valid) {
    GK_HIP(hipMemcpyAsync(tab->d_pair_gene, pair_gene, (size_t)n_valid, hipMemcpyHostToDevice, st));
    GK_HIP(hipMemcpyAsync(tab->d_pair_nh, pair_nh, (size_t)n_valid, hipMemcpyHostToDevice, st));
  }
  GK_HIP(hipStreamSynchronize(st));
  *out = tab;
  return GK_OK;
}

int gk_tab_get_info(gk_tab* tab, gk_tab_info* info) {
  gk_bind(tab ? tab->ctx : nullptr);
  GK_REQUIRE(tab && info, "null pointer");
  info->n_pairs = tab->n_pairs; info->n_valid = tab->n_valid; info->n_ids = tab->n_ids;
  info->n_novel = tab->n_novel; info->err_flags = tab->err_flags;
  info->d_pair_src = gk_addr(tab->d_pair_src); info->d_off = gk_addr(tab->d_off); info->d_ids = gk_addr(tab->d_ids);
  info->d_pair_gene = gk_addr(tab->d_pair_gene); info->d_pair_nh = gk_addr(tab->d_pair_nh);
  info->d_novel_key = gk_addr(tab->d_novel_key);
  return GK_OK;
}

int gk_tab_destroy(gk_tab* tab) {
  gk_bind(tab ? tab->ctx : nullptr);
  if (!tab) return GK_OK;
  gk_ctx* ctx = tab->ctx;
  gk_pool_free(ctx,tab->d_pair_src); gk_pool_free(ctx,tab->d_off); gk_pool_free(ctx,tab->d_ids);
// ... 49 lines not shown
```

kir_graph_amd/csrc/gk_typing.hip:

```cpp
#include <algorithm>

#include "gk_common.h"
#include "gk_lut.h"

namespace {

constexpr int kThreads = 256;
inline unsigned nblk(int64_t n, int t = kThreads) { return (unsigned)((n + t - 1) / t); }

template <bool kScatter>
__global__ __launch_bounds__(kThreads) void part_pass(const uint8_t* gene, const uint8_t* nh, int64_t n, int multiple,
                                                      int n_bins, int64_t n_tiles, uint32_t* hist, int32_t* out) {
  const int64_t i = (int64_t)blockIdx.x * kThreads + threadIdx.x;
  const int lane = threadIdx.x & 63;
  const int64_t tile = i >> 6;
  int bin = -1;
  if (i < n && (multiple || nh[i] == 1)) {
    bin = gene[i];
    if (bin >= n_bins) bin = -1;
  }
  uint64_t todo = __ballot(bin >= 0);
  while (todo) {
    const int leader = __ffsll((unsigned long long)todo) - 1;
    const int b = __shfl(bin, leader, 64);
// ... 8 lines not shown
}

__global__ void part_offsets(const uint32_t* hist, const uint32_t* total, int n_bins, int64_t n_tiles, uint32_t* goff) {
  const int b = blockIdx.x * blockDim.x + threadIdx.x;
  if (b < n_bins) goff[b] = hist[(int64_t)b * n_tiles];
  if (b == n_bins) goff[b] = *total;
}

__global__ __launch_bounds__(kThreads) void count_ids(const int32_t* __restrict__ rows, int64_t n_rows,
                                                      const uint32_t* __restrict__ off,
                                                      const uint32_t* __restrict__ ids,
                                                      const uint8_t* __restrict__ vflag, uint32_t* cnt_pos,
                                                      uint32_t* cnt_neg, int vbeg, int n_local) {
  extern __shared__ uint32_t hist[];
  for (int i = threadIdx.x; i < 2 * n_local; i += kThreads) hist[i] = 0;
  __syncthreads();
  constexpr int kGroup = 16;
  const int lane = threadIdx.x & (kGroup - 1);
  const int64_t group = ((int64_t)blockIdx.x * kThreads + threadIdx.x) / kGroup;
  const int64_t n_groups = ((int64_t)gridDim.x * kThreads) / kGroup;
  for (int64_t i = group; i < n_rows; i += n_groups) {
    const int64_t row = rows[i];
    const uint32_t b = off[4 * row], mid = off[4 * row + 2], e = off[4 * row + 4];
    for (uint32_t k = b + lane; k < e; k += kGroup) {
      const uint32_t v = ids[k];
      const bool positive = k < mid;
      if (vflag[v] & (positive ? 1 : 2)) continue;
      const uint32_t l = v - (uint32_t)vbeg;
      if (l < (uint32_t)n_local) atomicAdd(&hist[(positive ? 0 : n_local) + l], 1u);
      else atomicAdd(positive ? &cnt_pos[v] : &cnt_neg[v], 1u);
    }
  }
  __syncthreads();
  for (int i = threadIdx.x; i < 2 * n_local; i += kThreads) {
    const uint32_t c = hist[i];
    if (c) atomicAdd(i < n_local ? &cnt_pos[vbeg + i] : &cnt_neg[vbeg + i - n_local], c);
  }
}

__global__ __launch_bounds__(kThreads) void apply_correction(const uint32_t* cnt_pos, const uint32_t* cnt_neg,
                                                             int64_t n, uint8_t* vflag) {
  const int64_t v = (int64_t)blockIdx.x * kThreads + threadIdx.x;
  if (v >= n) return;
  const uint64_t p = cnt_pos[v], q = cnt_neg[v];
  if (p + q == 0) return;
  uint8_t f = vflag[v];
  if (p + q < 3) {
    f |= 3;
  } else {
    if (5 * p < p + q) f |= 1;
    if (5 * q < p + q) f |= 2;
  }
  vflag[v] = f;
}

__global__ __launch_bounds__(kThreads) void flag_nonempty(const int32_t* rows, int64_t n_rows, const uint32_t* off,
                                                          const uint32_t* ids, const uint8_t* vflag, uint32_t* flag,
                                                          uint32_t* zero, int n_zero) {
  const int64_t i = (int64_t)blockIdx.x * kThreads + threadIdx.x;
  if (zero && i < n_zero) zero[i] = 0;
  if (i >= n_rows) return;
  const int64_t row = rows[i];
  const uint32_t b = off[4 * row], mid = off[4 * row + 2], e = off[4 * row + 4];
  uint32_t alive = 0;
  for (uint32_t k = b; k < e && !alive; ++k) alive = !(vflag[ids[k]] & (k < mid ? 1 : 2));
  flag[i] = alive;
}

__global__ __launch_bounds__(kThreads) void flag_pairs(int64_t n_pairs, const uint32_t* __restrict__ off,
                                                       const uint32_t* __restrict__ ids, const uint8_t* __restrict__ vflag,
                                                       const uint8_t* __restrict__ maybe, uint8_t* __restrict__ alive) {
  const int64_t t = (int64_t)blockIdx.x * kThreads + threadIdx.x;
  const int64_t p = t >> 2;
  const uint32_t l = (uint32_t)t & 3u;
  uint32_t b = 0, mid = 0, e = 0;
  if (p < n_pairs && maybe[p]) { b = off[4 * p]; mid = off[4 * p + 2]; e = off[4 * p + 4]; }
  const int shift = (threadIdx.x & 63) & ~3;
  bool any = false;
  for (uint32_t k0 = b; k0 < e && !any; k0 += 4) {
    const uint32_t k = k0 + l;
    const bool mine = k < e && !(vflag[ids[k]] & (k < mid ? 1 : 2));
    any = ((__ballot(mine) >> shift) & 0xFull) != 0ull;
  }
  if (p < n_pairs && l == 0) alive[p] = any ? 1 : 0;
}

__global__ __launch_bounds__(kThreads) void gather_pair_flags(const int32_t* __restrict__ rows, int64_t n_rows,
                                                              const uint8_t* __restrict__ alive, uint32_t* __restrict__ flag,
                                                              uint32_t* zero, int n_zero) {
  const int64_t i = (int64_t)blockIdx.x * kThreads + threadIdx.x;
  if (zero && i < n_zero) zero[i] = 0;
  if (i < n_rows) flag[i] = alive[rows[i]];
}

__global__ __launch_bounds__(kThreads) void count_ids_genes(const int32_t* __restrict__ rows,
                                                            const int32_t* __restrict__ wg_gene,
                                                            const int64_t* __restrict__ wg_row0,
                                                            const int64_t* __restrict__ wg_row1,
                                                            const int32_t* __restrict__ gene_vbeg, int max_local,
                                                            const uint32_t* __restrict__ off,
                                                            const uint32_t* __restrict__ ids,
                                                            const uint8_t* __restrict__ vflag, uint32_t* cnt_pos,
                                                            uint32_t* cnt_neg, uint8_t* __restrict__ maybe) {
  extern __shared__ uint32_t hist[];
  const int g = wg_gene[blockIdx.x];
  const int vbeg = gene_vbeg[g];
// ... 621 lines not shown
  if (!nv) return GK_OK;
  uint32_t* cnt = gk_ptr<uint32_t>(d_cnt);
  uint32_t *flag = nullptr, *vals = nullptr;
  int32_t* ord = nullptr;
  GK_HIP(gk_pool_malloc(ctx, (void**)&flag, (size_t)nv * sizeof(uint32_t)));
  GK_HIP(gk_pool_malloc(ctx, (void**)&ord, (size_t)nv * sizeof(int32_t)));
  GK_KERNEL(flag_surviving, dim3(nblk(nv)), dim3(kThreads), 0, ctx->stream, cnt, cnt + nv,
                     gk_ptr<uint8_t>(d_vflag), nv, flag, gene, vbeg, vend, tab->n_var, tab->d_novel_key);
  int64_t n = 0;
  int rc = gk_compact(ctx, flag, nullptr, nv, ord, &n);
  if (rc == GK_OK && n > max_out) {
    gk_set_error("surviving-variant buffer too small (%lld > %lld)", (long long)n, (long long)max_out);
    rc = GK_ERR_CAPACITY;
  }
  if (rc == GK_OK && n) {
    GK_HIP(gk_pool_malloc(ctx, (void**)&vals, (size_t)(2 * n) * sizeof(uint32_t)));
    GK_KERNEL(gather_surviving, dim3(nblk(n)), dim3(kThreads), 0, ctx->stream, ord, n, cnt, cnt + nv,
                       gk_ptr<uint8_t>(d_vflag), vals);
    GK_HIP(gk_fetch_queue(ctx, ord_out, ord, (size_t)n * sizeof(int32_t)));
    GK_HIP(gk_fetch_queue(ctx, pos_out, vals, (size_t)n * sizeof(uint32_t)));
    GK_HIP(gk_fetch_queue(ctx, neg_out, vals + n, (size_t)n * sizeof(uint32_t)));
    GK_HIP(gk_fetch_wait(ctx));
    gk_pool_free(ctx, vals);
  }
  gk_pool_free(ctx, flag);
  gk_pool_free(ctx, ord);
  if (rc == GK_OK) *n_out = n;
  return rc;
}

int gk_variant_surviving(gk_ctx* ctx, gk_tab* tab, gk_dptr d_cnt, gk_dptr d_vflag, int64_t max_out, int32_t* ord_out,
                         uint32_t* pos_out, uint32_t* neg_out, int64_t* n_out) {
  return variant_surviving(ctx, tab, d_cnt, d_vflag, max_out, ord_out, pos_out, neg_out, n_out, -1, 0, 0);
}

int gk_variant_surviving_gene(gk_ctx* ctx, gk_tab* tab, gk_dptr d_cnt, gk_dptr d_vflag, int32_t gene, int32_t vbeg,
                              int32_t vend, int64_t max_out, int32_t* ord_out, uint32_t* pos_out, uint32_t* neg_out,
                              int64_t* n_out) {
  GK_REQUIRE(gene >= 0 && vend >= vbeg, "bad gene range");
  return variant_surviving(ctx, tab, d_cnt, d_vflag, max_out, ord_out, pos_out, neg_out, n_out, gene, vbeg, vend);
}

namespace {
struct Survivors {
  int64_t max_out = 0;
  int32_t* ord = nullptr;
  uint32_t *pos = nullptr, *neg = nullptr;
  int64_t* n_out = nullptr;
  uint64_t* novel_key = nullptr;
};
}

static int sample_prepare(gk_ctx* ctx, gk_tab* tab, int32_t multiple, gk_dptr d_vflag, gk_dptr d_cnt, gk_dptr d_rows,
                          int64_t* gene_off_out, const Survivors* surv, bool keep_vflag = false, int rounds = 1);

int gk_sample_prepare(gk_ctx* ctx, gk_tab* tab, int32_t multiple, gk_dptr d_vflag, gk_dptr d_cnt, gk_dptr d_rows,
                      int64_t* gene_off_out) {
  return sample_prepare(ctx, tab, multiple, d_vflag, d_cnt, d_rows, gene_off_out, nullptr);
}

int gk_sample_prepare_all(gk_ctx* ctx, gk_tab* tab, int32_t multiple, gk_dptr d_vflag, gk_dptr d_cnt, gk_dptr d_rows,
                          int64_t* gene_off_out, int64_t max_out, int32_t* ord_out, uint32_t* pos_out, uint32_t* neg_out,
                          int64_t* n_out, uint64_t* novel_key_out) {
  GK_REQUIRE(ord_out && pos_out && neg_out && n_out && max_out >= 0, "null pointer");
  Survivors s;
  s.max_out = max_out; s.ord = ord_out; s.pos = pos_out; s.neg = neg_out; s.n_out = n_out; s.novel_key = novel_key_out;
  return sample_prepare(ctx, tab, multiple, d_vflag, d_cnt, d_rows, gene_off_out, &s);
}

int gk_sample_prepare_exon(gk_ctx* ctx, gk_tab* tab, int32_t multiple, gk_dptr d_vflag, gk_dptr d_cnt, gk_dptr d_rows,
                           int64_t* gene_off_out, int64_t max_out, int32_t* ord_out, uint32_t* pos_out, uint32_t* neg_out,
                           int64_t* n_out) {
  GK_REQUIRE(ord_out && pos_out && neg_out && n_out && max_out >= 0, "null pointer");
  Survivors s;
  s.max_out = max_out; s.ord = ord_out; s.pos = pos_out; s.neg = neg_out; s.n_out = n_out; s.novel_key = nullptr;
  return sample_prepare(ctx, tab, multiple, d_vflag, d_cnt, d_rows, gene_off_out, &s, true, 2);
}

static int sample_prepare(gk_ctx* ctx, gk_tab* tab, int32_t multiple, gk_dptr d_vflag, gk_dptr d_cnt, gk_dptr d_rows,
                          int64_t* gene_off_out, const Survivors* surv, bool keep_vflag, int rounds) {
  gk_bind(ctx);
  GK_REQUIRE(ctx && tab && tab->idx && d_vflag && d_cnt && d_rows && gene_off_out, "null pointer");
  if (surv) *surv->n_out = 0;
  const int n_gene = tab->idx->n_gene;
  const int64_t nv = (int64_t)tab->n_var + tab->n_novel;
  hipStream_t st = ctx->stream;
  for (int g = 0; g <= n_gene; ++g) gene_off_out[g] = 0;
  if (!keep_vflag) GK_HIP(hipMemsetAsync(gk_ptr<void>(d_vflag), 0, (size_t)std::max<int64_t>(nv, 1), st));
  GK_HIP(hipMemsetAsync(gk_ptr<void>(d_cnt), 0, (size_t)std::max<int64_t>(2 * nv, 1) * sizeof(uint32_t), st));
  auto novel_only = [&]() -> int {
    if (surv && surv->novel_key && tab->n_novel > 0)
      GK_HIP(gk_fetch(ctx, surv->novel_key, tab->d_novel_key, (size_t)tab->n_novel * sizeof(uint64_t)));
    return GK_OK;
  };
  if (tab->n_valid == 0) return novel_only();
  gk_tab::GenePartition& part = tab->part[multiple ? 1 : 0];
  {
    std::lock_guard<std::mutex> lock(tab->part_mutex);
    if (part.gene_off.empty()) {
      int rc = build_partition(ctx, tab, multiple);
      if (rc) { part.gene_off.clear(); return rc; }
    }
  }
  GK_REQUIRE((int)part.gene_off.size() >= n_gene + 1, "partition does not cover the genes");
  const int64_t n_rows = part.gene_off[n_gene];
  if (n_rows == 0) return novel_only();
  std::vector<int32_t> wg_gene;
  std::vector<int64_t> wg_row0, wg_row1, goff(part.gene_off.begin(), part.gene_off.begin() + n_gene + 1);
  const int64_t per_wg = std::max<int64_t>(64, (n_rows + 2047) / 2048);
  int max_span = 0;
  for (int g = 0; g < n_gene; ++g) {
    max_span = std::max(max_span, tab->idx->gene_vbeg[g + 1] - tab->idx->gene_vbeg[g]);
    for (int64_t r = goff[g]; r < goff[g + 1]; r += per_wg) {
      wg_gene.push_back(g);
      wg_row0.push_back(r);
      wg_row1.push_back(std::min(goff[g + 1], r + per_wg));
    }
  }
  const int max_local = std::min(max_span, 60 * 1024 / 8);
  const size_t n_wg = wg_gene.size();
  char* d_tab = nullptr;
  const size_t o_row0 = (n_wg * sizeof(int32_t) + 15) / 16 * 16, o_row1 = o_row0 + n_wg * sizeof(int64_t),
               o_goff = o_row1 + n_wg * sizeof(int64_t), tab_bytes = o_goff + (size_t)(n_gene + 1) * sizeof(int64_t);
  {
    std::vector<char> packed(tab_bytes);
    memcpy(packed.data(), wg_gene.data(), n_wg * sizeof(int32_t));
    memcpy(packed.data() + o_row0, wg_row0.data(), n_wg * sizeof(int64_t));
    memcpy(packed.data() + o_row1, wg_row1.data(), n_wg * sizeof(int64_t));
    memcpy(packed.data() + o_goff, goff.data(), (size_t)(n_gene + 1) * sizeof(int64_t));
    GK_HIP(gk_pool_malloc(ctx, (void**)&d_tab, tab_bytes));
    GK_HIP(gk_send(ctx, d_tab, packed.data(), tab_bytes));
  }
  uint32_t* cnt = gk_ptr<uint32_t>(d_cnt);
  uint8_t* vflag = gk_ptr<uint8_t>(d_vflag);
  uint8_t *maybe = nullptr, *alive = nullptr;
  GK_HIP(gk_pool_malloc(ctx, (void**)&maybe, (size_t)tab->n_valid));
  GK_HIP(gk_pool_malloc(ctx, (void**)&alive, (size_t)tab->n_valid));
  GK_HIP(hipMemsetAsync(maybe, 0, (size_t)tab->n_valid, st));
  for (int round = 0; round < rounds; ++round) {
    if (round) GK_HIP(hipMemsetAsync(cnt, 0, (size_t)(2 * nv) * sizeof(uint32_t), st));
    GK_PROF(ctx, "count_ids_genes",
            GK_KERNEL(count_ids_genes, dim3((unsigned)n_wg), dim3(kThreads), (size_t)max_local * 8 + kThreads * sizeof(uint32_t), st, part.d_rows,
                      (const int32_t*)d_tab, (const int64_t*)(d_tab + o_row0), (const int64_t*)(d_tab + o_row1),
                      tab->idx->d_gene_vbeg, max_local, tab->d_off, tab->d_ids, vflag, cnt, cnt + nv,
                      round == rounds - 1 ? maybe : (uint8_t*)nullptr));
    GK_PROF(ctx, "apply_correction", GK_KERNEL(apply_correction, dim3(nblk(nv)), dim3(kThreads), 0, st, cnt, cnt + nv, nv, vflag));
  }
  uint32_t *flag = nullptr, *kept = nullptr;
  GK_HIP(gk_pool_malloc(ctx, (void**)&flag, (size_t)n_rows * sizeof(uint32_t)));
  GK_HIP(gk_pool_malloc(ctx, (void**)&kept, (size_t)n_gene * sizeof(uint32_t)));
  GK_PROF(ctx, "flag_pairs", GK_KERNEL(flag_pairs, dim3(nblk(4 * (int64_t)tab->n_valid)), dim3(kThreads), 0, st, (int64_t)tab->n_valid,
                                   tab->d_off, tab->d_ids, vflag, maybe, alive));
  GK_PROF(ctx, "gather_pair_flags", GK_KERNEL(gather_pair_flags, dim3(nblk(std::max<int64_t>(n_rows, n_gene))), dim3(kThreads), 0, st,
                                          part.d_rows, n_rows, alive, flag, kept, n_gene));
  GK_PROF(ctx, "count_flags_per_gene", GK_KERNEL(count_flags_per_gene, dim3((unsigned)n_gene, kFlagSlices), dim3(kThreads), 0, st, flag,
                                      (const int64_t*)(d_tab + o_goff), kept));
  GK_HIP(hipGetLastError());
  std::vector<void*> temps{flag, kept, d_tab, alive, maybe};
  auto done = [&](int code) {
    for (void* t : temps) gk_pool_free(ctx, t);
    return code;
  };
  uint32_t* d_total = nullptr;
  int rc = gk_compact_enqueue(ctx, flag, part.d_rows, n_rows, gk_ptr<int32_t>(d_rows), &d_total, temps);
  if (rc) return done(rc);
  uint32_t total = 0, n_surv = 0;
  std::vector<uint32_t> host((size_t)n_gene);
  bool queued = gk_fetch_queue(ctx, &total, d_total, sizeof(uint32_t)) == hipSuccess &&
                gk_fetch_queue(ctx, host.data(), kept, (size_t)n_gene * sizeof(uint32_t)) == hipSuccess;
  if (queued && surv && nv > 0) {
    const int64_t cap = std::min<int64_t>(nv, surv->max_out);
    uint32_t *sflag = nullptr, *vals = nullptr, *d_n = nullptr;
    int32_t* ord = nullptr;
    auto take = [&](void** p, size_t bytes) {
      if (gk_pool_malloc(ctx, p, bytes) != hipSuccess) return false;
      temps.push_back(*p);
      return true;
    };
    if (!take((void**)&sflag, (size_t)nv * sizeof(uint32_t)) || !take((void**)&ord, (size_t)nv * sizeof(int32_t)) ||
        !take((void**)&vals, (size_t)std::max<int64_t>(2 * cap, 1) * sizeof(uint32_t))) {
      gk_fetch_cancel(ctx);
      gk_set_error("out of device memory for the surviving tallies");
      return done(GK_ERR_HIP);
    }
    GK_KERNEL(flag_surviving, dim3(nblk(nv)), dim3(kThreads), 0, st, cnt, cnt + nv, vflag, nv, sflag, -1, 0, 0, tab->n_var,
              tab->d_novel_key);
    rc = gk_compact_enqueue(ctx, sflag, nullptr, nv, ord, &d_n, temps);
    if (rc) { gk_fetch_cancel(ctx); return done(rc); }
    if (cap > 0) {
      GK_KERNEL(gather_surviving_queued, dim3(nblk(cap)), dim3(kThreads), 0, st, ord, d_n, cap, cnt, cnt + nv, vflag, vals);
      queued = gk_fetch_queue(ctx, surv->ord, ord, (size_t)cap * sizeof(int32_t)) == hipSuccess &&
               gk_fetch_queue(ctx, surv->pos, vals, (size_t)cap * sizeof(uint32_t)) == hipSuccess &&
               gk_fetch_queue(ctx, surv->neg, vals + cap, (size_t)cap * sizeof(uint32_t)) == hipSuccess;
    }
    queued = queued && gk_fetch_queue(ctx, &n_surv, d_n, sizeof(uint32_t)) == hipSuccess;
    if (queued && surv->novel_key && tab->n_novel > 0)
      queued = gk_fetch_queue(ctx, surv->novel_key, tab->d_novel_key, (size_t)tab->n_novel * sizeof(uint64_t)) == hipSuccess;
  }
// ... 107 lines not shown
```

kir_graph_amd/engine.py:

```python
from __future__ import annotations

import ctypes as C
import os
import threading
from typing import NamedTuple

import numpy as np

from . import _lib
from ._lib import Device, DeviceBuffer, DeviceSlice, TabInfo, check, lib
from .index import GkIndex, KEY_POS_SHIFT, KEY_TYP_SHIFT, KEY_VAL_MASK
from .msa2hisat import Variant

TYPE_OF_RANK = {0: "insertion", 1: "single", 2: "deletion"}


def _i32(a) -> np.ndarray:
    return np.ascontiguousarray(a, dtype=np.int32)


def searchMode() -> str:
    mode = os.environ.get("GK_SEARCH", "bound")
    if mode not in ("bound", "exact"):
        raise ValueError(f"GK_SEARCH={mode!r}: expected 'bound' or 'exact'")
# ... 23 lines not shown
class PreparedSample(NamedTuple):
    vflag: DeviceBuffer
    cnt: DeviceBuffer
    rows: DeviceBuffer
    off: np.ndarray
    surviving: Surviving

    def gene(self, g: int, vbeg: int, vend: int, dev: Device | None = None) -> PreparedGene:
        a, b = int(self.off[g]), int(self.off[g + 1])
        return PreparedGene(DeviceSlice(self.rows, a, b - a, dev), b - a, self.vflag, self.cnt, (g, vbeg, vend),
                            self.surviving.ofGene(g))


def _groupByGene(gene_of: np.ndarray, o: np.ndarray, p: np.ndarray, q: np.ndarray, n_genes: int) -> Surviving:
    order = np.argsort(gene_of, kind="stable")
    bounds = np.searchsorted(gene_of[order], np.arange(n_genes + 1)).astype(np.int64)
    return Surviving(np.ascontiguousarray(o[order], dtype=np.int32), np.ascontiguousarray(p[order], dtype=np.uint32),
                     np.ascontiguousarray(q[order], dtype=np.uint32), bounds)


class DeviceIndex:

    def __init__(self, dev: Device, index: GkIndex):
        self.dev, self.host = dev, index
        h = C.c_void_p()
        key = np.ascontiguousarray(index.key, dtype=np.uint64)
        vbeg = _i32(index.gene_vbeg)
        check(lib().gk_index_create(dev.ctx, key.ctypes.data, len(key), vbeg.ctypes.data, len(index.genes),
                                    C.byref(h)))
        self.handle = h
        self.masks = [dev.put(t.mask) for t in index.tables]

    def close(self) -> None:
        if self.handle:
            lib().gk_index_destroy(self.handle)
            self.handle = None


class Tabulation:

    def __init__(self, dindex: DeviceIndex, mates, novel_base: int = 0, dev: Device | None = None,
                 correction: tuple[np.ndarray, np.ndarray] | None = None,
                 spill: tuple[np.ndarray, np.ndarray] | None = None):
        self.dev, self.dindex = dev or dindex.dev, dindex
        self._spill, self._correction = spill, correction
        if isinstance(mates, np.ndarray):
            assert mates.dtype == _lib.MATE_DTYPE
            self.mates = self.dev.put(mates)
        elif hasattr(mates, "toDevice"):
            self.mates = mates.toDevice(self.dev)
        else:
            self.mates = mates
        self.n_pairs = self.mates.size // 2
        h = C.c_void_p()
        d_table = d_pos0 = None
        if correction is not None:
            table, pos0 = correction
            assert table.dtype == np.uint8 and table.shape == (int(pos0[-1]), 5) and len(pos0) == len(dindex.host.genes) + 1
            d_table = self.dev.put(np.ascontiguousarray(table).reshape(-1) if table.size else np.zeros(1, np.uint8))
            d_pos0 = self.dev.put(np.ascontiguousarray(pos0, dtype=np.int64))
        if spill is not None and len(spill[1]):
            wide = np.ascontiguousarray(spill[0], dtype=_lib.MATE_WIDE_DTYPE)
            which = np.ascontiguousarray(spill[1], dtype=np.int64)
            assert len(wide) == 2 * len(which)
            check(lib().gk_tabulate_spilled(self.dev.ctx, dindex.handle, self.mates.ptr, self.n_pairs,
                                            d_table.ptr if d_table else 0, d_pos0.ptr if d_pos0 else 0,
                                            wide.ctypes.data, which.ctypes.data, len(which), C.byref(h)))
        elif correction is None:
            check(lib().gk_tabulate(self.dev.ctx, dindex.handle, self.mates.ptr, self.n_pairs, C.byref(h)))
        else:
            check(lib().gk_tabulate_corrected(self.dev.ctx, dindex.handle, self.mates.ptr, self.n_pairs,
                                              d_table.ptr, d_pos0.ptr, C.byref(h)))
        self.handle = h
        info = TabInfo()
        check(lib().gk_tab_get_info(h, C.byref(info)))
        self.info = info
        self.n_valid, self.n_ids, self.n_novel = int(info.n_valid), int(info.n_ids), int(info.n_novel)
        self.novel_base = novel_base
        if info.err_flags & 1:
            raise AssertionError("variant window has left > right (graphkir/hisat2.py:744)")
        self._novel_keys = None
        if self.dev.call_log is not None:
            self.dev.call_log.append(("tab_count", self.n_pairs, self.n_valid, self.n_ids))

    @property
    def n_var_total(self) -> int:
        override = getattr(self, "_id_names", None)
        if override is not None:
            return len(override)
        return self.dindex.host.n_variant + self.n_novel

    def close(self) -> None:
        if self.handle and not getattr(self, "_borrowed", False):
            for prep in (getattr(self, "_prepared", None) or {}).values():
                for b in (prep.vflag, prep.cnt, prep.rows):
                    b.free()
            self._prepared = {}
            lib().gk_tab_destroy(self.handle)
        self.handle = None

    def prepared(self, dev: Device, multiple: bool = False, exon: bool = False) -> PreparedSample | None:
        if self.dindex is None or not self.info.d_pair_src:
            return None
        root = getattr(self, "_root", self)
        lock = root.__dict__.setdefault("_prep_lock", threading.Lock())
        store = root.__dict__.setdefault("_prepared", {})
        key = (bool(multiple), True) if exon else bool(multiple)
        with lock:
            prep = store.get(key)
            if prep is None:
                host = self.dindex.host
                nv = max(self.n_var_total, 1)
                if exon:
                    flags = np.full(nv, 3, dtype=np.uint8)
                    flags[:host.n_variant][host.in_exon.astype(bool)] = 0
                    vflag = dev.put(flags)
                else:
                    vflag = dev.alloc(nv, np.uint8)
                cnt = dev.alloc(2 * nv, np.uint32)
                rows = dev.alloc(max(self.n_valid, 1), np.int32)
                off = np.zeros(len(host.genes) + 1, dtype=np.int64)
                o, p, q = (np.empty(nv, dtype=t) for t in (np.int32, np.uint32, np.uint32))
                n_surv = C.c_int64()
                args = (dev.ctx, self.handle, int(multiple), vflag.ptr, cnt.ptr, rows.ptr, off.ctypes.data, nv,
                        o.ctypes.data, p.ctypes.data, q.ctypes.data, C.byref(n_surv))
                if exon:
                    check(lib().gk_sample_prepare_exon(*args))
                else:
                    want_novel = self._novel_keys is None and self.n_novel > 0
                    novel_keys = np.empty(self.n_novel, dtype=np.uint64) if want_novel else None
                    check(lib().gk_sample_prepare_all(*args, novel_keys.ctypes.data if want_novel else None))
                    if want_novel:
                        self._novel_keys = root._novel_keys = novel_keys
                o, p, q = o[:n_surv.value], p[:n_surv.value], q[:n_surv.value]
                gene_of = np.searchsorted(host.gene_vbeg, o, side="right") - 1
                if not exon and len(o) and int(o[-1]) >= host.n_variant:
                    is_novel = o >= host.n_variant
                    gene_of[is_novel] = (self.novelKeys()[o[is_novel] - host.n_variant] >> np.uint64(56)).astype(gene_of.dtype)
                prep = store[key] = PreparedSample(vflag, cnt, rows, off, _groupByGene(gene_of, o, p, q, len(host.genes)))
        return prep

    @staticmethod
    def survivingOfGene(prep: PreparedSample, g: int):
        return prep.surviving.ofGene(g)

    def on(self, dev: Device) -> "Tabulation":
        if dev is self.dev:
            return self
        import copy
        other = copy.copy(self)
        other.dev = dev
        other._borrowed = True
        other._root = getattr(self, "_root", self)
        return other

    def offsets(self) -> np.ndarray:
        return self.dev.view(self.info.d_off, 4 * self.n_valid + 1, np.uint32)

    def ids(self) -> np.ndarray:
        return self.dev.view(self.info.d_ids, self.n_ids, np.uint32)

    def pairSrc(self) -> np.ndarray:
        return self.dev.view(self.info.d_pair_src, self.n_valid, np.int32)

    def pairGene(self) -> np.ndarray:
        return self.dev.view(self.info.d_pair_gene, self.n_valid, np.uint8)

    def pairNH(self) -> np.ndarray:
        return self.dev.view(self.info.d_pair_nh, self.n_valid, np.uint8)

    def novelKeys(self) -> np.ndarray:
        if self._novel_keys is None:
            self._novel_keys = self.dev.view(self.info.d_novel_key, self.n_novel, np.uint64)
        return self._novel_keys

    def novelVariants(self, ins_strings: list[str]) -> list[Variant]:
        genes = self.dindex.host.genes
        out = []
        for rank, k in enumerate(self.novelKeys().tolist()):
            ref = genes[k >> 56]
# ... 406 lines not shown
```

kir_graph_amd/hisat2.py:

```python
from __future__ import annotations

import json
import re
from dataclasses import asdict, dataclass, field, fields as dataclass_fields
from typing import Iterable, Iterator, TypedDict

import ctypes as C
import numpy as np

from . import _lib
from ._lib import Device, check, lib
from .engine import DeviceIndex, Tabulation
from .index import GkIndex, getVariants, readExons
from .msa2hisat import Variant
from .packed import packPairs
from .utils import logger


@dataclass
class PairRead:

    l_sam: str = ""
    r_sam: str = ""
    multiple: int = 1
# ... 151 lines not shown

    def asDict(self) -> ReadsAndVariantsData:
        return {"variants": self.variants, "reads": self.reads()}

    @classmethod
    def fromHost(cls, dev: Device, data: ReadsAndVariantsData) -> "SampleData":
        known = sorted(v for v in data["variants"] if not str(v.id).startswith("nv"))
        novel = [v for v in data["variants"] if str(v.id).startswith("nv")]
        genes = sorted(set(v.ref for v in data["variants"]) | set(r.backbone for r in data["reads"]))
        index = GkIndex.fromVariants(known, genes=genes)
        ordinal = {str(v.id): i for i, v in enumerate(index.variants + novel)}
        reads = data["reads"]
        n = len(reads)
        off = np.zeros(4 * n + 1, dtype=np.uint32)
        flat: list[int] = []
        for i, r in enumerate(reads):
            for k, lst in enumerate((r.lpv, r.rpv, r.lnv, r.rnv)):
                flat.extend(ordinal[v] for v in lst)
                off[4 * i + k + 1] = len(flat)
        ids = np.array(flat, dtype=np.uint32)
        gene = np.array([index.gene_id[r.backbone] for r in reads], dtype=np.uint8)
        nh = np.array([min(int(r.multiple), 255) for r in reads], dtype=np.uint8)
        dindex = DeviceIndex(dev, index)
        tab = Tabulation.__new__(Tabulation)
        tab.dev, tab.dindex, tab.mates, tab.n_pairs = dev, dindex, None, n
        h = C.c_void_p()
        check(lib().gk_tab_from_csr(dev.ctx, len(ordinal), n, off.ctypes.data, ids.ctypes.data if len(ids) else None,
                                    gene.ctypes.data if n else None, nh.ctypes.data if n else None, C.byref(h)))
        tab.handle = h
        info = _lib.TabInfo()
        check(lib().gk_tab_get_info(h, C.byref(info)))
        tab.info = info
        tab.n_valid, tab.n_ids = n, int(info.n_ids)
        tab.n_novel, tab.novel_base, tab._novel_keys = len(novel), 0, None
        tab._id_names = [str(v.id) for v in index.variants + novel]
        tab._variant_src = index.variants + novel
        self = cls(tab, index, novel)
        self._reads = list(reads)
        return self


class ParkedRecords:

    def __init__(self, data: "SampleData"):
        import ctypes as C
        tab = data.tab
        if tab.mates is None:
            raise ValueError("the packed records of the sample have been released already")
        self.dev, self.dindex, self.index = tab.dev, tab.dindex, data.index
        self.ins_strings = data.ins_strings
        self.n_pairs, self.novel_base = tab.n_pairs, tab.novel_base
        self.expect = (tab.n_valid, tab.n_ids, tab.n_novel)
        self.spill, self.correction = getattr(tab, "_spill", None), getattr(tab, "_correction", None)
        ptr, nbytes = C.c_uint64(), C.c_int64()
        check(lib().gk_mates_compact(self.dev.ctx, tab.mates.ptr, 2 * self.n_pairs, C.byref(ptr), C.byref(nbytes)))
        self.ptr, self.nbytes = ptr.value, int(nbytes.value)
        self.dev.sync()
        tab.mates.free()
        tab.mates = None
        tab.close()

    def restore(self) -> "SampleData":
        if not self.ptr:
            raise ValueError("restored already")
        mates = self.dev.alloc(2 * self.n_pairs, _lib.MATE_DTYPE)
        check(lib().gk_mates_expand(self.dev.ctx, self.ptr, 2 * self.n_pairs, mates.ptr))
        self.release()
        tab = Tabulation(self.dindex, mates, novel_base=self.novel_base, dev=self.dev, spill=self.spill,
                         correction=self.correction)
        if (tab.n_valid, tab.n_ids, tab.n_novel) != self.expect:
            raise AssertionError(f"second tabulation differs from the first: {(tab.n_valid, tab.n_ids, tab.n_novel)} "
                                 f"!= {self.expect}")
        return SampleData(tab, self.index, None, ins_strings=self.ins_strings)

    def release(self) -> None:
        if self.ptr:
            lib().gk_free(self.dev.ctx, self.ptr)
            self.ptr = 0

    def __del__(self):
        try:
            self.release()
        except Exception:
            pass


COMPACT_FORMAT = "graphkir-variant-csr-1"


def indexFingerprint(index: GkIndex) -> np.ndarray:
    key = index.key.astype(np.uint64)
    return np.array([len(key), int(key.sum(dtype=np.uint64)), int(np.bitwise_xor.reduce(key)) if len(key) else 0],
                    dtype=np.uint64)


def writeCompact(data: SampleData, filename: str, index_ref: str = "", background=None):
    tab = data.tab
    if getattr(tab, "_variant_src", None) is not None:
        raise ValueError("compact files are written from tabulations made against an index")
    path = filename if filename.endswith(".npz") else filename + ".npz"
    fields = dict(
        format=np.array(COMPACT_FORMAT), index_ref=np.array(index_ref), fingerprint=indexFingerprint(data.index),
        genes=np.array(data.index.genes), off=tab.offsets(), ids=tab.ids(), pair_gene=tab.pairGene(),
        pair_nh=tab.pairNH(), novel_key=tab.novelKeys(), novel_base=np.array(tab.novel_base),
        ins_strings=np.array(data.ins_strings if data.ins_strings else [""]),
        n_ins=np.array(len(data.ins_strings or [])))
    if background is None:
        np.savez(path, **fields)
        return None
    return background.submit(np.savez, path, **fields)


RECORDS_FORMAT = "graphkir-records-1"


def writeCompactRecords(compact, pack: dict, novel_base: int, index: GkIndex, filename: str, index_ref: str = "",
                        background=None):
    path = filename if filename.endswith(".npz") else filename + ".npz"
    spill = pack["counts"].get("spill")
    strings = pack["strings"]
    fields = dict(
        format=np.array(RECORDS_FORMAT), index_ref=np.array(index_ref), fingerprint=indexFingerprint(index),
        genes=np.array(index.genes), words=np.asarray(compact.words), n_mates=np.array(compact.n_mates),
        novel_base=np.array(novel_base), ins_strings=np.array(strings if strings else [""]),
        n_ins=np.array(len(strings or [])),
        spill_wide=(np.ascontiguousarray(spill[0]).view(np.uint8).reshape(-1) if spill is not None else np.zeros(0, np.uint8)),
        spill_pair=(np.ascontiguousarray(spill[1], dtype=np.int64) if spill is not None else np.zeros(0, np.int64)))
    if background is None:
        np.savez(path, **fields)
# ... 242 lines not shown
```

kir_graph_amd/packed.py:

```python
from __future__ import annotations

import re

import numpy as np

from ._lib import MATE_DTYPE, CIG_M, CIG_I, CIG_D, CIG_S, NM_ABSENT, MAX_CIG, MAX_MM, MAX_INS, MAX_EV
from .index import GkIndex

_CIGAR = re.compile(r"(\d+)(\w)")
_MDTOK = re.compile(r"\d+|.")
_NH = re.compile(r"NH:i:(\d+)")
MAX_OPLEN = 4095


class PackCapacityError(ValueError):
    """A filter-passing record does not fit the fixed-size device record."""


class InsTable:

    def __init__(self, index: GkIndex):
        self.strings = list(index.ins_strings)
        self.ids = dict(index.ins_id)
        self.n_index = len(self.strings)

    def intern(self, s: str) -> int:
        i = self.ids.get(s)
        if i is None:
            i = len(self.strings)
            self.ids[s] = i
            self.strings.append(s)
        return i


def _decodeTags(cols: list[str]):
    nm = None
    md = zs = None
    for c in cols:
        if c.startswith("NM"):
            nm = int(c[5:])
        elif md is None and c.startswith("MD"):
            md = c[5:]
        elif zs is None and c.startswith("Zs"):
            zs = c[5:]
    return nm, md, zs


def _passes(flag: int, nm) -> bool:
    return bool(flag & 2) and nm is not None and nm <= 4


def _walkText(pos0: int, cigar: str, seq: str, md_s: str | None, zs_s: str | None, table: InsTable):
    md = [int(t) if t.isdigit() else t for t in _MDTOK.findall(md_s)] if md_s is not None else []
    zs = [(int(a), b) for a, b, _ in (x.split("|") for x in zs_s.split(","))] if zs_s else []
    ops: list[tuple[int, int]] = []
# ... 368 lines not shown
        np.add.at(rec["n_mm"], ss, 1)
        is_i = kind == EV_INS
        i_rank = _rankWithin(rep, is_i)
        si = slot_of[is_i]
        rec["ins"][si, i_rank[is_i]] = ins_map[eval_[is_i]]
        np.add.at(rec["n_ins"], si, 1)
        is_x = ~is_s
        x_rank = _rankWithin(rep, is_x)
        sx = slot_of[is_x]
        xoff = off[is_x]
        xk = kind[is_x]
        xlen = np.where(xk == EV_DEL, eval_[is_x], 0)
        if sample.ins_strings:
            ilen = np.array([len(s) for s in sample.ins_strings], dtype=np.int64)
            xlen_ins = np.where(xk == EV_INS, ilen[np.where(xk == EV_INS, eval_[is_x], 0)], 0)
        else:
            xlen_ins = np.zeros(len(xk), dtype=np.int64)
        prev_end = np.zeros(len(xk), dtype=np.int64)
        same = np.zeros(len(xk), dtype=bool)
        if len(xk) > 1:
            same[1:] = sx[1:] == sx[:-1]
            prev_end[1:] = np.where(same[1:], (xoff + xlen)[:-1], 0)
        gap = xoff - prev_end
        xr = x_rank[is_x]
        cig[sx, 2 * xr] = ((gap << 4) | CIG_M).astype(np.uint16)
        oplen = np.where(xk == EV_DEL, xlen, xlen_ins)
        cig[sx, 2 * xr + 1] = ((oplen << 4) | np.where(xk == EV_DEL, CIG_D, CIG_I)).astype(np.uint16)
        n_x = np.bincount(sx, minlength=n_m)
        last_end = np.zeros(n_m, dtype=np.int64)
        np.maximum.at(last_end, sx, xoff + xlen)
    else:
        n_x = np.zeros(n_m, dtype=np.int64)
        last_end = np.zeros(n_m, dtype=np.int64)
    fin = span.astype(np.int64) - last_end
    t = np.nonzero(todo)[0]
    cig[t, 2 * n_x[t]] = ((fin[t] << 4) | CIG_M).astype(np.uint16)
    rec["n_cig"][t] = (2 * n_x[t] + 1).astype(np.uint8)
    if np.any(fin[t] <= 0):
        raise PackCapacityError("synthetic mate ends in an indel")
    return rec, table


def _rankWithin(group: np.ndarray, sel: np.ndarray) -> np.ndarray:
    n = len(group)
    if not n:
        return np.zeros(0, dtype=np.int64)
    before = np.cumsum(sel) - sel
    start = np.ones(n, dtype=bool)
    start[1:] = group[1:] != group[:-1]
    first = np.maximum.accumulate(np.where(start, np.arange(n), 0))
    return (before - before[first]).astype(np.int64)


class CompactMates:

    def __init__(self, records: np.ndarray, threads: int = 4):
        import ctypes as C
        from ._lib import MATE_DTYPE, check, lib, pinnedEmpty
        assert records.dtype == MATE_DTYPE
        records = np.ascontiguousarray(records)
        self.n_mates = len(records)
        n_words = C.c_int64()
        check(lib().gk_mates_compact_size(records.ctypes.data, self.n_mates, threads, C.byref(n_words)))
        self.words = pinnedEmpty(self.n_mates + 1 + n_words.value, np.uint32)
        check(lib().gk_mates_compact_host(records.ctypes.data, self.n_mates, threads, self.words.ctypes.data, len(self.words)))

    @property
    def nbytes(self) -> int:
        return int(self.words.nbytes)

    def toDevice(self, dev, wait: bool = False):
        import ctypes as C
        from ._lib import MATE_DTYPE, check, lib
        compact = dev.alloc(len(self.words), np.uint32)
        check(lib().gk_h2d_async(dev.ctx, compact.ptr, C.c_void_p(self.words.ctypes.data), self.words.nbytes))
        mates = dev.alloc(self.n_mates, MATE_DTYPE)
        check(lib().gk_mates_expand(dev.ctx, compact.ptr, self.n_mates, mates.ptr))
        compact.free()
        if wait:
            dev.sync()
        return mates
```

kir_graph_amd/roofmodel.py:

```python
from __future__ import annotations

HBM_PEAK_GBS = 8000.0
TILE = 32
N_SIMD = 256 * 4
NOMINAL_HZ = 2.4e9

ISSUE_CYCLES = {"v_mul_f64": 4.50, "v_add_f64": 4.26, "v_max_f64": 4.19, "v_bfe_i32": 4.43, "v_bfi_b32": 4.56,
                "v_sad_u8": 4.49}
GUIDE_CYCLES = {"v_mul_f64": 4.0, "v_add_f64": 4.0, "v_max_f64": 4.0, "v_bfe_i32": 2.0, "v_bfi_b32": 2.0, "v_sad_u8": 2.0}
SEQUENCE_CYCLES = {"compat_kernel": 5.81}
KERNEL_OPS = {
    "compat_kernel": ("v_bfe_i32", "v_bfi_b32", "v_bfi_b32", "v_mul_f64"),
    "minsum_sad": ("v_sad_u8",),
    "maxsum_chunks": ("v_max_f64", "v_add_f64"),
}


def laneOpsPeak(kernel: str, table: dict[str, float] = ISSUE_CYCLES) -> float:
    ops = KERNEL_OPS[kernel]
    return len(ops) * 64 * N_SIMD * NOMINAL_HZ / sum(table[o] for o in ops)


def symmetricOutputs(n: int) -> int:
    total = 0
    for t0 in range(0, n, TILE):
        rows = min(TILE, n - t0)
        total += rows * (n - t0)
    return total


def maxsumLaunch(n_rows: int, n_sets: int, c_prev: int, n_cols: int, n_prev_cols: int,
                 symmetric: bool = False) -> tuple[float, float]:
    by = 8.0 * n_rows * (n_cols + n_prev_cols) + 8.0 * n_sets * n_cols
    outputs = symmetricOutputs(n_cols) if symmetric else n_sets * n_cols
    return by, 2.0 * n_rows * outputs


def minsumLaunch(n_rows: int, n_sets: int, n_cols: int, n_prev_cols: int, symmetric: bool = False
                 ) -> tuple[float, float]:
    outputs = symmetricOutputs(n_cols) if symmetric else n_sets * n_cols
    return 1.0 * n_rows * (n_cols + n_prev_cols) + 4.0 * n_sets * n_cols, n_rows * outputs / 4.0


def compatLaunch(n_rows: int, n_allele: int, n_ids: float, out_bytes: int = 8) -> tuple[float, float]:
    return 4.0 * n_ids + 16.0 * n_rows + float(out_bytes + 1) * n_rows * n_allele, 4.0 * n_ids * n_allele


def tabLaunch(n_pairs: int, n_valid: int, n_ids: int) -> tuple[float, float]:
    return 256.0 * n_pairs + 4.0 * n_ids + 22.0 * n_valid, 0.0


def setsumLaunch(n_rows: int, n_sets: int, c: int, n_distinct: int) -> tuple[float, float]:
    return 8.0 * n_rows * n_distinct + 8.0 * n_sets * (c + 1), float(n_rows) * n_sets * (c + 1)


def emSetsLaunch(n_rows: int, n_ids: float, set_words: int) -> tuple[float, float]:
    return 24.0 * n_rows + 4.0 * n_ids + 4.0 * set_words, 0.0


def emVerifyLaunch(set_words: int) -> tuple[float, float]:
    return 4.0 * set_words, 0.0


def _priced(kernel: str, calls: list[tuple]) -> tuple[float, float, str, float]:
    by = ops = 0.0
    bound, peak = "hbm", 0.0
    for c in calls:
        if kernel == "maxsum_chunks":
            b, o = maxsumLaunch(*c[1:7])
            bound, peak = "valu", laneOpsPeak("maxsum_chunks")
        elif kernel == "colsum_chunks":
            b, o = 8.0 * c[1] * c[4] + 8.0 * c[4], 0.0
        elif kernel == "em_sets_groups":
            b, o = emSetsLaunch(*c[1:4])
        elif kernel == "em_sets_verify":
            b, o = emVerifyLaunch(c[3])
        elif kernel == "minsum_sad":
            b, o = minsumLaunch(*c[1:6])
            bound, peak = "valu", laneOpsPeak("minsum_sad")
        elif kernel == "compat_kernel":
            b, o = compatLaunch(*c[1:5])
            bound, peak = "valu", laneOpsPeak("compat_kernel")
        elif kernel == "compat_rows8":
            b, o = compatLaunch(*c[1:5])[0], 0.0
        elif kernel == "tab_count":
            b, o = tabLaunch(*c[1:4])
        elif kernel in ("fraction_chunks", "setsum_leaves"):
            b, o = setsumLaunch(*c[1:5])
        else:
            return 0.0, 0.0, "hbm", 0.0
        by += b
        ops += o
    return by, ops, bound, peak


def summarise(call_log: list[tuple], kernel: str, total_ms: float, launches: int) -> dict:
    calls = [c for c in call_log if c[0] == kernel]
    base = {"kernel": kernel, "bound": "hbm", "achieved": None, "peak": HBM_PEAK_GBS, "unit": "GB/s",
            "frac": None, "traffic": None, "launches": launches, "avg_launch_ms": total_ms / max(launches, 1)}
    if not calls or total_ms <= 0:
        return base
    by, ops, bound, peak = _priced(kernel, calls)
    if by <= 0:
        return base
    sec = total_ms / 1e3
    gbs = by / sec / 1e9
    hbm = {"achieved": gbs, "peak": HBM_PEAK_GBS, "unit": "GB/s", "frac": gbs / HBM_PEAK_GBS}
    out = dict(base)
    out["algorithmic_bytes_per_launch"] = by / max(launches, 1)
    if bound == "valu":
        tops = ops / sec / 1e12
        unit = {"maxsum_chunks": "Tops/s f64 (max+add)", "minsum_sad": "T lane-ops/s (v_sad_u8, 4 reads each)",
                "compat_kernel": "T lane-ops/s (4 VALU per id and allele)"}.get(kernel, "T lane-ops/s")
        guide = laneOpsPeak(kernel, GUIDE_CYCLES)
        out.update({"bound": "valu", "achieved": tops, "peak": peak / 1e12, "unit": unit, "frac": ops / sec / peak,
                    "peak_guide": guide / 1e12, "frac_guide": ops / sec / guide,
                    "issue_cycles": {o: ISSUE_CYCLES[o] for o in KERNEL_OPS[kernel]},
                    "algorithmic_ops_per_launch": ops / max(launches, 1), "hbm": hbm,
                    "note": "VALU-issue bound (ordered f64 products / a (max,+) or (min,+) contraction).  `peak` = the "
                            "kernel's own instruction mix issued back to back at the MEASURED cost of each instruction "
                            "(tools/valu_rate.hip at 8 waves per SIMD, profiles/r03_valu_rate.txt: cycles of a 2.4 GHz "
                            "clock per wave64 instruction and SIMD in `issue_cycles`); `peak_guide` / `frac_guide` price "
                            "the same mix at the guide's 2 cycles per 32-bit and 4 per float64 instruction.  The HBM "
                            "roof is shown beside it; symmetric launches are credited with the triangle of tiles they "
                            "compute"})
        if kernel in SEQUENCE_CYCLES:
            seq = 64 * N_SIMD * NOMINAL_HZ / SEQUENCE_CYCLES[kernel]
            out["peak_sequence"] = seq / 1e12
            out["frac_sequence"] = ops / sec / seq
            out["note"] += (".  `peak_sequence` / `frac_sequence`: the same instructions at the rate measured for them "
                            "as the sequence the kernel issues (eight independent chains per wave, 8 waves per SIMD)")
    else:
        out.update(hbm)
        out["bound"] = "hbm"
    return out


def dominant(prof: dict[str, tuple[int, float]], call_log: list[tuple]) -> dict:
    if not prof:
# ... 49 lines not shown
```

kir_graph_amd/samtools_utils.py:

```python
from __future__ import annotations

import numpy as np
import pandas as pd

from ._lib import check, lib
from .external_tools import runTool


def bam2Depth(file_bam: str, file_depth: str, get_all: bool = True) -> None:
    args = ["samtools", "depth"] + (["-aa"] if get_all else []) + [file_bam, "-o", file_depth]
    runTool("samtools", args)


def readSamtoolsDepth(depth_filename: str) -> pd.DataFrame:
    return pd.read_csv(depth_filename, sep="\t", header=None, names=["gene", "pos", "depth"])


def readLocusLengths(index: str) -> dict[str, int]:
    out = {}
    with open(index + ".locus") as f:
        for line in f:
            cols = line.split("\t")
            out[cols[0]] = int(cols[4])
    return out


def depthOfSample(data, gene_len: dict[str, int], file_depth: str | None = None, multiple: bool = False,
                  want_frame: bool = True) -> pd.DataFrame | None:
    import ctypes as C
    tab = data.tab
    genes = data.index.genes
    lens = np.array([gene_len[g] for g in genes], dtype=np.int64)
    off = np.zeros(len(genes) + 1, dtype=np.int64)
    np.cumsum(lens, out=off[1:])
    depth = np.empty(int(off[-1]), dtype=np.uint32)
    check(lib().gk_depth(tab.dev.ctx, tab.handle, tab.mates.ptr, int(multiple), off.ctypes.data, len(genes),
                         depth.ctypes.data))
    if file_depth:
        names = (C.c_char_p * len(genes))(*[g.encode() for g in genes])
        check(lib().gk_depth_write_tsv(file_depth.encode(), names, off.ctypes.data, len(genes), depth.ctypes.data))
    if not want_frame:
        return None
    return pd.DataFrame({
        "gene": np.repeat(np.array(genes, dtype=object), lens),
        "pos": np.concatenate([np.arange(1, n + 1) for n in lens]) if len(lens) else np.zeros(0, np.int64),
        "depth": depth.astype(np.int64),
    })
```

Before: 474.3 million.

## Keep mate records compact on device and tabulate directly from compact words

Tabulation and depth kernels now read variable-length compact mate words (with a per-mate offset array) instead of expanding them into fixed 256-byte records. The compact run for each block is staged into the same LDS budget, and full records are expanded lazily only when a legacy path asks for a pointer. This is meant to cut the HBM traffic and the expand pass in the record-bound tabulation. It also adds a reuse of full-gene counts in exon prepare and a gc.freeze in the cohort runner. The cost is extra indexing arithmetic and more complex record lifetime handling.

```diff
diff --git a/include/graphkir_hip.h b/include/graphkir_hip.h
--- a/include/graphkir_hip.h
+++ b/include/graphkir_hip.h
@@ -118,6 +118,10 @@
 int gk_tabulate_spilled(gk_ctx* ctx, gk_index* idx, gk_dptr d_mates, int64_t n_pairs, gk_dptr d_corr,
                         gk_dptr d_gene_pos0, const gk_mate_wide* wide, const int64_t* spill_pair, int64_t n_spill,
                         gk_tab** out);
+#define GK_COMPACT_STAGE_WORDS 4352
+int gk_tabulate_compact(gk_ctx* ctx, gk_index* idx, gk_dptr d_compact, int64_t n_pairs, gk_dptr d_corr,
+                        gk_dptr d_gene_pos0, const gk_mate_wide* wide, const int64_t* spill_pair, int64_t n_spill,
+                        gk_tab** out);
 int gk_tab_from_csr(gk_ctx* ctx, int32_t n_var_total, int64_t n_valid, const uint32_t* off, const uint32_t* ids,
                     const uint8_t* pair_gene, const uint8_t* pair_nh, gk_tab** out);
 int gk_tab_get_info(gk_tab* tab, gk_tab_info* info);
@@ -146,6 +150,9 @@
 int gk_sample_prepare_exon(gk_ctx* ctx, gk_tab* tab, int32_t multiple, gk_dptr d_vflag, gk_dptr d_cnt, gk_dptr d_rows,
                            int64_t* gene_off_out, int64_t max_out, int32_t* ord_out, uint32_t* pos_out, uint32_t* neg_out,
                            int64_t* n_out);
+int gk_sample_prepare_exon_from(gk_ctx* ctx, gk_tab* tab, int32_t multiple, gk_dptr d_vflag, gk_dptr d_cnt, gk_dptr d_rows,
+                                int64_t* gene_off_out, int64_t max_out, int32_t* ord_out, uint32_t* pos_out,
+                                uint32_t* neg_out, int64_t* n_out, gk_dptr d_cnt_full);
 
 int gk_compat(gk_ctx* ctx, gk_tab* tab, gk_dptr d_rows, int64_t n_rows, gk_dptr d_vflag,
               int32_t vbeg, int32_t vend, gk_dptr d_mask, int32_t words, int32_t n_allele, int32_t keep_empty,
@@ -326,6 +333,8 @@
 
 int gk_depth(gk_ctx* ctx, gk_tab* tab, gk_dptr d_mates, int32_t multiple, const int64_t* gene_off,
              int32_t n_gene, uint32_t* depth_out);
+int gk_depth_compact(gk_ctx* ctx, gk_tab* tab, gk_dptr d_compact, int32_t multiple, const int64_t* gene_off,
+                     int32_t n_gene, uint32_t* depth_out);
 
 int gk_depth_write_tsv(const char* path, const char* const* genes, const int64_t* gene_off, int32_t n_genes,
                        const uint32_t* depth);
diff --git a/kir_graph_amd/_lib.py b/kir_graph_amd/_lib.py
--- a/kir_graph_amd/_lib.py
+++ b/kir_graph_amd/_lib.py
@@ -38,6 +38,7 @@
 CIG_M, CIG_I, CIG_D, CIG_S = 0, 1, 2, 4
 NM_ABSENT = 255
 MAX_CIG, MAX_MM, MAX_INS, MAX_EV = 14, 16, 6, 22
+COMPACT_STAGE_WORDS = 4352
 
 
 class GeneJob(C.Structure):
@@ -109,6 +110,8 @@
                                      C.c_void_p, C.c_void_p, C.c_int64, C.POINTER(C.c_void_p)]),
     "gk_tabulate_corrected": (C.c_int, [C.c_void_p, C.c_void_p, C.c_uint64, C.c_int64, C.c_uint64, C.c_uint64,
                                         C.POINTER(C.c_void_p)]),
+    "gk_tabulate_compact": (C.c_int, [C.c_void_p, C.c_void_p, C.c_uint64, C.c_int64, C.c_uint64, C.c_uint64,
+                                     C.c_void_p, C.c_void_p, C.c_int64, C.POINTER(C.c_void_p)]),
     "gk_tab_from_csr": (C.c_int, [C.c_void_p, C.c_int32, C.c_int64, C.c_void_p, C.c_void_p, C.c_void_p, C.c_void_p,
                                   C.POINTER(C.c_void_p)]),
     "gk_tab_get_info": (C.c_int, [C.c_void_p, C.POINTER(TabInfo)]),
@@ -180,6 +183,7 @@
     "gk_packer_spill_records": (C.c_int, [C.c_void_p, C.c_void_p, C.c_void_p]),
     "gk_packer_string": (C.c_char_p, [C.c_void_p, C.c_int64]),
     "gk_depth": (C.c_int, [C.c_void_p, C.c_void_p, C.c_uint64, C.c_int32, C.c_void_p, C.c_int32, C.c_void_p]),
+    "gk_depth_compact": (C.c_int, [C.c_void_p, C.c_void_p, C.c_uint64, C.c_int32, C.c_void_p, C.c_int32, C.c_void_p]),
     "gk_depth_write_tsv": (C.c_int, [C.c_char_p, C.c_void_p, C.c_void_p, C.c_int32, C.c_void_p]),
     "gk_cn_fit": (C.c_int, [C.c_void_p, C.c_void_p, C.c_void_p, C.c_int32, C.c_void_p, C.c_int32, C.c_void_p,
                             C.c_int32, C.c_int32, C.c_double, C.c_void_p]),
@@ -218,6 +222,8 @@
                                  C.POINTER(C.c_int32)]),
     "gk_sample_prepare_exon": (C.c_int, [C.c_void_p, C.c_void_p, C.c_int32, C.c_uint64, C.c_uint64, C.c_uint64, C.c_void_p,
                                          C.c_int64, C.c_void_p, C.c_void_p, C.c_void_p, C.POINTER(C.c_int64)]),
+    "gk_sample_prepare_exon_from": (C.c_int, [C.c_void_p, C.c_void_p, C.c_int32, C.c_uint64, C.c_uint64, C.c_uint64, C.c_void_p,
+                                              C.c_int64, C.c_void_p, C.c_void_p, C.c_void_p, C.POINTER(C.c_int64), C.c_uint64]),
     "gk_sample_em": (C.c_int, [C.c_void_p, C.c_void_p, C.c_void_p, C.c_int32, C.c_int32, C.c_double, C.c_void_p, C.c_void_p]),
     "gk_mates_compact": (C.c_int, [C.c_void_p, C.c_uint64, C.c_int64, C.POINTER(C.c_uint64), C.POINTER(C.c_int64)]),
     "gk_mates_expand": (C.c_int, [C.c_void_p, C.c_uint64, C.c_int64, C.c_uint64]),
diff --git a/kir_graph_amd/cohort.py b/kir_graph_amd/cohort.py
--- a/kir_graph_amd/cohort.py
+++ b/kir_graph_amd/cohort.py
@@ -105,7 +105,8 @@
     else:
         per_read = 9.2 * mean_alleles * (2 if method.startswith(("exonfirst", "pv_exonfirst")) else 1)
     lists = 4.0 * int(tab.n_ids) + 48.0 * n
-    records = 256.0 * int(tab.n_pairs) if getattr(tab, "mates", None) is not None else 0.0
+    mates = getattr(tab, "mates", None)
+    records = float(getattr(mates, "nbytes", 256.0 * int(tab.n_pairs))) if mates is not None else 0.0
     return int(1.15 * per_read * n + lists + records)
 
 
@@ -141,6 +142,8 @@
         import threading
         self._room = threading.Condition()
         self._inflight_bytes, self._budget = 0, None
+        import gc
+        gc.freeze()
 
     def _admit(self, data) -> int:
         need = sampleFootprint(data, self.method)
@@ -200,6 +203,8 @@
         if self._pool is not None:
             self._pool.shutdown(wait=True)
             self._pool = None
+        import gc
+        gc.unfreeze()
 
     def __enter__(self):
         return self
diff --git a/kir_graph_amd/csrc/gk_depth.hip b/kir_graph_amd/csrc/gk_depth.hip
--- a/kir_graph_amd/csrc/gk_depth.hip
+++ b/kir_graph_amd/csrc/gk_depth.hip
@@ -1,10 +1,17 @@
+#include <cstddef>
+
 #include "gk_common.h"
 
 namespace {
 
 constexpr int kThreads = 256;
+constexpr int kInsWord = offsetof(gk_mate, ins) / 4;
+static_assert(offsetof(gk_mate, cig) == 12 && offsetof(gk_mate, pos0) == 0, "gk_mate layout");
 
+template <bool kCompact>
 __global__ __launch_bounds__(kThreads) void depth_mark(const gk_mate* __restrict__ mates,
+                                                       const uint32_t* __restrict__ c_off,
+                                                       const uint32_t* __restrict__ c_words,
                                                        const gk_mate_wide* __restrict__ wide,
                                                        const int32_t* __restrict__ pair_src,
                                                        const uint8_t* __restrict__ pair_nh, int64_t n_valid,
@@ -14,10 +21,12 @@
   if (t >= 2 * n_valid) return;
   const int64_t i = t >> 1;
   if (!multiple && pair_nh[i] != 1) return;
-  const gk_mate& m = mates[2 * (int64_t)pair_src[i] + (t & 1)];
-  if (m.ref >= n_gene) return;
-  const int64_t base = gene_off[m.ref], len = gene_off[m.ref + 1] - base;
-  int64_t cur = m.pos0;
+  const int64_t at = 2 * (int64_t)pair_src[i] + (t & 1);
+  const uint32_t* w = kCompact ? c_words + c_off[at] : reinterpret_cast<const uint32_t*>(mates + at);
+  const uint32_t ref = (w[1] >> 16) & 0xFFu, n_ops = (w[2] >> 8) & 0xFFu;
+  if ((int)ref >= n_gene) return;
+  const int64_t base = gene_off[ref], len = gene_off[ref + 1] - base;
+  int64_t cur = w[0];
   auto run = [&](uint32_t op, uint32_t n) {
     if (op == GK_CIG_M) {
       const int64_t a = cur < 0 ? 0 : cur, b = cur + n > len ? len : cur + n;
@@ -30,15 +39,20 @@
       cur += n;
     }
   };
-  if (m.n_cig == GK_SPILLED) {
+  if (n_ops == GK_SPILLED) {
     if (!wide) return;
-    const gk_mate_wide& x = wide[2 * (int64_t)m.ins[0] + (t & 1)];
+    const uint32_t slot = kCompact ? w[3] : w[kInsWord];
+    const gk_mate_wide& x = wide[2 * (int64_t)slot + (t & 1)];
     const int n_cig = x.n_cig < GK_WIDE_CIG ? x.n_cig : GK_WIDE_CIG;
     for (int c = 0; c < n_cig; ++c) run(x.cig[c] & 15u, x.cig[c] >> 4);
     return;
   }
-  const int n_cig = m.n_cig < GK_MAX_CIG ? m.n_cig : GK_MAX_CIG;
-  for (int c = 0; c < n_cig; ++c) run(m.cig[c] & 15u, m.cig[c] >> 4);
+  const int n_cig = n_ops < GK_MAX_CIG ? (int)n_ops : GK_MAX_CIG;
+  for (int c = 0; c < n_cig; ++c) {
+    const uint32_t x = w[3 + (c >> 1)];
+    const uint32_t cg = (c & 1) ? (x >> 16) : (x & 0xFFFFu);
+    run(cg & 15u, cg >> 4);
+  }
 }
 
 __global__ __launch_bounds__(kThreads) void depth_finish(const uint32_t* excl, const uint32_t* diff, int64_t n,
@@ -49,11 +63,12 @@
 
 }
 
-extern "C" int gk_depth(gk_ctx* ctx, gk_tab* tab, gk_dptr d_mates, int32_t multiple, const int64_t* gene_off,
-                        int32_t n_gene, uint32_t* depth_out) {
+static int depth_of(gk_ctx* ctx, gk_tab* tab, gk_dptr d_mates, gk_dptr d_compact, int32_t multiple, const int64_t* gene_off,
+                    int32_t n_gene, uint32_t* depth_out) {
   gk_bind(ctx);
   GK_REQUIRE(ctx && tab && gene_off && depth_out && n_gene > 0, "bad depth arguments");
   GK_REQUIRE(tab->d_pair_src, "depth needs a tabulation made from packed records");
+  GK_REQUIRE(tab->n_valid == 0 || d_mates || d_compact, "depth needs the sample's records");
   const int64_t total = gene_off[n_gene];
   hipStream_t st = ctx->stream;
   uint32_t *diff = nullptr, *scan = nullptr;
@@ -63,10 +78,16 @@
   GK_HIP(gk_pool_malloc(ctx, (void**)&d_off, (size_t)(n_gene + 1) * sizeof(int64_t)));
   GK_HIP(hipMemsetAsync(diff, 0, (size_t)(total + 1) * sizeof(uint32_t), st));
   GK_HIP(hipMemcpyAsync(d_off, gene_off, (size_t)(n_gene + 1) * sizeof(int64_t), hipMemcpyHostToDevice, st));
-  if (tab->n_valid)
-    GK_KERNEL(depth_mark, dim3((unsigned)((2 * tab->n_valid + kThreads - 1) / kThreads)), dim3(kThreads), 0, st,
-                       gk_ptr<const gk_mate>(d_mates), tab->d_wide, tab->d_pair_src, tab->d_pair_nh, tab->n_valid, multiple, d_off,
-                       n_gene, diff);
+  if (tab->n_valid) {
+    const dim3 grid((unsigned)((2 * tab->n_valid + kThreads - 1) / kThreads));
+    const uint32_t* c_off = gk_ptr<const uint32_t>(d_compact);
+    if (c_off)
+      GK_KERNEL(depth_mark<true>, grid, dim3(kThreads), 0, st, (const gk_mate*)nullptr, c_off, c_off + 2 * tab->n_pairs + 1,
+                tab->d_wide, tab->d_pair_src, tab->d_pair_nh, tab->n_valid, multiple, d_off, n_gene, diff);
+    else
+      GK_KERNEL(depth_mark<false>, grid, dim3(kThreads), 0, st, gk_ptr<const gk_mate>(d_mates), c_off, c_off, tab->d_wide,
+                tab->d_pair_src, tab->d_pair_nh, tab->n_valid, multiple, d_off, n_gene, diff);
+  }
   GK_HIP(hipMemcpyAsync(scan, diff, (size_t)(total + 1) * sizeof(uint32_t), hipMemcpyDeviceToDevice, st));
   int rc = gk_scan_u32(ctx, scan, total + 1, nullptr);
   if (rc) return rc;
@@ -80,3 +101,14 @@
   gk_pool_free(ctx, d_off);
   return GK_OK;
 }
+
+extern "C" int gk_depth(gk_ctx* ctx, gk_tab* tab, gk_dptr d_mates, int32_t multiple, const int64_t* gene_off,
+                        int32_t n_gene, uint32_t* depth_out) {
+  return depth_of(ctx, tab, d_mates, 0, multiple, gene_off, n_gene, depth_out);
+}
+
+extern "C" int gk_depth_compact(gk_ctx* ctx, gk_tab* tab, gk_dptr d_compact, int32_t multiple, const int64_t* gene_off,
+                                int32_t n_gene, uint32_t* depth_out) {
+  GK_REQUIRE(d_compact || (tab && tab->n_valid == 0), "null compact records");
+  return depth_of(ctx, tab, 0, d_compact, multiple, gene_off, n_gene, depth_out);
+}
diff --git a/kir_graph_amd/csrc/gk_tabulate.hip b/kir_graph_amd/csrc/gk_tabulate.hip
--- a/kir_graph_amd/csrc/gk_tabulate.hip
+++ b/kir_graph_amd/csrc/gk_tabulate.hip
@@ -1,4 +1,5 @@
 #include <algorithm>
+#include <type_traits>
 #include <vector>
 
 #include "gk_common.h"
@@ -67,6 +68,55 @@
   __device__ bool passes() const { return (flag() & 2u) && nm() != GK_NM_ABSENT && nm() <= 4u; }
 };
 static_assert(kCigWord + GK_MAX_CIG / 2 <= kHeadWords, "the CIGAR lies in the staged head");
+
+constexpr int kStageWords = GK_COMPACT_STAGE_WORDS;
+static_assert(kStageWords == kThreads * kHeadLd, "the compact run is staged in the LDS budget of the staged heads");
+struct CompactView {
+  static constexpr int kCapCig = GK_MAX_CIG, kCapMm = GK_MAX_MM, kCapIns = GK_MAX_INS, kCapEv = kMaxEv;
+  const uint32_t* run;
+  const uint32_t* g;
+  uint32_t base;
+  uint32_t o_mm, o_ins;
+  uint32_t n_ins_w;
+  uint32_t h0, h1, h2;
+  __device__ uint32_t word(uint32_t i) const { return i < (uint32_t)kStageWords ? run[i] : g[i]; }
+  __device__ void open(uint32_t at) {
+    base = at;
+    h0 = word(at); h1 = word(at + 1); h2 = word(at + 2);
+    const uint32_t nc = (h2 >> 8) & 0xFFu;
+    const bool sp = nc == GK_SPILLED;
+    const uint32_t n_cw = sp ? 0u : (min(nc, (uint32_t)GK_MAX_CIG) + 1u) / 2u;
+    const uint32_t n_mw = sp ? 0u : min((h2 >> 16) & 0xFFu, (uint32_t)GK_MAX_MM);
+    n_ins_w = sp ? 1u : min(h2 >> 24, (uint32_t)GK_MAX_INS);
+    o_mm = at + kCigWord + n_cw;
+    o_ins = o_mm + n_mw;
+  }
+  __device__ bool spilled() const { return n_cig() == GK_SPILLED; }
+  __device__ uint32_t pos0() const { return h0; }
+  __device__ uint32_t flag() const { return h1 & 0xFFFFu; }
+  __device__ uint32_t ref() const { return (h1 >> 16) & 0xFFu; }
+  __device__ uint32_t nm() const { return h2 & 0xFFu; }
+  __device__ uint32_t n_cig() const { return (h2 >> 8) & 0xFFu; }
+  __device__ uint32_t n_mm() const { return (h2 >> 16) & 0xFFu; }
+  __device__ uint32_t cig(int i) const {
+    const uint32_t x = word(base + kCigWord + ((uint32_t)i >> 1));
+    return (i & 1) ? (x >> 16) : (x & 0xFFFFu);
+  }
+  __device__ uint32_t mm_off(int i) const { return word(o_mm + (uint32_t)i) & 0xFFFFu; }
+  __device__ uint32_t mm_base(int i) const { return (word(o_mm + (uint32_t)i) >> 16) & 0xFFu; }
+  __device__ uint32_t ins(int i) const {
+    const bool has = (uint32_t)i < n_ins_w;
+    const uint32_t x = word(has ? o_ins + (uint32_t)i : base);
+    return has ? x : 0u;
+  }
+  __device__ bool passes() const { return (flag() & 2u) && nm() != GK_NM_ABSENT && nm() <= 4u; }
+};
+
+__device__ inline void stage_run(const uint32_t* g, uint32_t n_run, uint32_t* run) {
+  const uint32_t n = min(n_run, (uint32_t)kStageWords);
+  for (uint32_t i = threadIdx.x; i < n; i += kThreads) run[i] = g[i];
+  __syncthreads();
+}
 
 struct WideView {
   static constexpr int kCapCig = GK_WIDE_CIG, kCapMm = GK_WIDE_MM, kCapIns = GK_WIDE_INS, kCapEv = GK_WIDE_EVENTS;
@@ -455,7 +505,9 @@
   return kept;
 }
 
-__global__ __launch_bounds__(kThreads) void tab_count(const gk_mate* mates, int64_t n_mates, IndexView ix,
+template <bool kCompact>
+__global__ __launch_bounds__(kThreads) void tab_count(const gk_mate* mates, const uint32_t* __restrict__ c_off,
+                                                      const uint32_t* __restrict__ c_words, int64_t n_mates, IndexView ix,
                                                       NovelTable nt, uint32_t* cnt ,
                                                       uint32_t* valid , int* err_flags,
                                                       uint4* ev_save ,
@@ -465,10 +517,20 @@
                                                       uint32_t* mask_more ) {
   __shared__ uint32_t rec[kThreads * kHeadLd];
   const int64_t m0 = (int64_t)blockIdx.x * kThreads;
-  stage_heads(mates, m0, n_mates, rec);
   const int64_t m = m0 + threadIdx.x;
   const bool in = m < n_mates;
-  const HeadView r{rec + threadIdx.x * kHeadLd, reinterpret_cast<const uint32_t*>(mates + (in ? m : 0))};
+  typename std::conditional<kCompact, CompactView, HeadView>::type r;
+  if constexpr (kCompact) {
+    const uint32_t run0 = c_off[m0], run1 = c_off[min<int64_t>(m0 + kThreads, n_mates)];
+    const uint32_t at = c_off[in ? m : m0] - run0;
+    stage_run(c_words + run0, run1 - run0, rec);
+    r.run = rec; r.g = c_words + run0;
+    r.open(at);
+  } else {
+    stage_heads(mates, m0, n_mates, rec);
+    r.w = rec + threadIdx.x * kHeadLd;
+    r.g = reinterpret_cast<const uint32_t*>(mates + (in ? m : 0));
+  }
   EvRow ev{{0u, 0u, 0u, 0u}, ev_more + (in ? m : 0) * kEvMore, nt.keys};
   const bool ok = in && r.passes() && !r.spilled();
   const bool ok_other = __shfl_xor((int)ok, 1, 64) != 0;
@@ -713,7 +775,8 @@
     if (negative_kept(ix.key[i], i, ix, EvView{evw}, wk.n, wk.any_n, wk.right)) ids[at++] = (uint32_t)i;
 }
 
-__global__ __launch_bounds__(kThreads) void gather_pairs(const gk_mate* mates, const int32_t* pair_src, int64_t n_valid,
+__global__ __launch_bounds__(kThreads) void gather_pairs(const gk_mate* mates, const uint32_t* c_off, const uint32_t* c_words,
+                                                         const int32_t* pair_src, int64_t n_valid,
                                                          const uint32_t* off_in, uint32_t* off_out, uint8_t* gene,
                                                          uint8_t* nh, uint32_t total) {
   const int64_t i = (int64_t)blockIdx.x * kThreads + threadIdx.x;
@@ -725,7 +788,7 @@
   const int64_t p = pair_src[i];
 #pragma unroll
   for (int k = 0; k < 4; ++k) off_out[4 * i + k] = off_in[4 * p + k];
-  const uint32_t w1 = reinterpret_cast<const uint32_t*>(mates + 2 * p)[1];
+  const uint32_t w1 = mates ? reinterpret_cast<const uint32_t*>(mates + 2 * p)[1] : c_words[c_off[2 * p] + 1u];
   gene[i] = (uint8_t)((w1 >> 16) & 0xFFu);
   nh[i] = (uint8_t)(w1 >> 24);
 }
@@ -894,13 +957,29 @@
   return gk_tabulate_spilled(ctx, idx, d_mates_p, n_pairs, d_corr, d_gene_pos0, nullptr, nullptr, 0, out);
 }
 
-static int tabulate_with_table(gk_ctx* ctx, gk_index* idx, gk_dptr d_mates_p, int64_t n_pairs, gk_dptr d_corr,
+static int tabulate_with_table(gk_ctx* ctx, gk_index* idx, gk_dptr d_mates_p, gk_dptr d_compact, int64_t n_pairs, gk_dptr d_corr,
                                gk_dptr d_gene_pos0, const gk_mate_wide* wide, const int64_t* spill_pair,
                                int64_t n_spill, uint32_t log2cap, bool* table_too_small, gk_tab** out);
+static int tabulate_sample(gk_ctx* ctx, gk_index* idx, gk_dptr d_mates_p, gk_dptr d_compact, int64_t n_pairs, gk_dptr d_corr,
+                           gk_dptr d_gene_pos0, const gk_mate_wide* wide, const int64_t* spill_pair, int64_t n_spill,
+                           gk_tab** out);
 
 int gk_tabulate_spilled(gk_ctx* ctx, gk_index* idx, gk_dptr d_mates_p, int64_t n_pairs, gk_dptr d_corr,
                         gk_dptr d_gene_pos0, const gk_mate_wide* wide, const int64_t* spill_pair, int64_t n_spill,
                         gk_tab** out) {
+  return tabulate_sample(ctx, idx, d_mates_p, 0, n_pairs, d_corr, d_gene_pos0, wide, spill_pair, n_spill, out);
+}
+
+int gk_tabulate_compact(gk_ctx* ctx, gk_index* idx, gk_dptr d_compact, int64_t n_pairs, gk_dptr d_corr,
+                        gk_dptr d_gene_pos0, const gk_mate_wide* wide, const int64_t* spill_pair, int64_t n_spill,
+                        gk_tab** out) {
+  GK_REQUIRE(d_compact, "null compact records");
+  return tabulate_sample(ctx, idx, 0, d_compact, n_pairs, d_corr, d_gene_pos0, wide, spill_pair, n_spill, out);
+}
+
+static int tabulate_sample(gk_ctx* ctx, gk_index* idx, gk_dptr d_mates_p, gk_dptr d_compact, int64_t n_pairs, gk_dptr d_corr,
+                           gk_dptr d_gene_pos0, const gk_mate_wide* wide, const int64_t* spill_pair, int64_t n_spill,
+                           gk_tab** out) {
   uint32_t log2cap = 16;
   while ((1ull << log2cap) < (uint64_t)(2 * std::max<int64_t>(n_pairs, 0)) && log2cap < 22) ++log2cap;
   log2cap = (uint32_t)std::min<long>(30, std::max<long>(4, gk_test_hook_value("novel_log2cap", (long)log2cap)));
@@ -908,15 +987,15 @@
   while ((1ull << log2max) < (uint64_t)(2 * std::max<int64_t>(n_pairs, 0)) * GK_WIDE_EVENTS * 2 && log2max < 30) ++log2max;
   for (;;) {
     bool too_small = false;
-    const int rc = tabulate_with_table(ctx, idx, d_mates_p, n_pairs, d_corr, d_gene_pos0, wide, spill_pair, n_spill, log2cap,
-                                       &too_small, out);
+    const int rc = tabulate_with_table(ctx, idx, d_mates_p, d_compact, n_pairs, d_corr, d_gene_pos0, wide, spill_pair, n_spill,
+                                       log2cap, &too_small, out);
     if (!too_small) return rc;
     if (log2cap >= log2max) return rc;
     log2cap = std::min(log2cap + 3, log2max);
   }
 }
 
-static int tabulate_with_table(gk_ctx* ctx, gk_index* idx, gk_dptr d_mates_p, int64_t n_pairs, gk_dptr d_corr,
+static int tabulate_with_table(gk_ctx* ctx, gk_index* idx, gk_dptr d_mates_p, gk_dptr d_compact, int64_t n_pairs, gk_dptr d_corr,
                                gk_dptr d_gene_pos0, const gk_mate_wide* wide, const int64_t* spill_pair,
                                int64_t n_spill, uint32_t log2cap, bool* table_too_small, gk_tab** out) {
   gk_bind(ctx);
@@ -929,6 +1008,9 @@
   GK_REQUIRE(n_pairs < (1ll << 26), "more than 2^26 pairs per call");
   const gk_mate* mates = gk_ptr<const gk_mate>(d_mates_p);
   const int64_t n_mates = 2 * n_pairs;
+  const uint32_t* c_off = gk_ptr<const uint32_t>(d_compact);
+  const uint32_t* c_words = c_off ? c_off + n_mates + 1 : nullptr;
+  GK_REQUIRE(n_mates == 0 || mates || c_off, "no records");
   hipStream_t st = ctx->stream;
   gk_tab* tab = new gk_tab();
   tab->ctx = ctx; tab->idx = idx; tab->n_pairs = n_pairs; tab->n_var = idx->n_var;
@@ -960,8 +1042,12 @@
                      gk_ptr<uint8_t>(d_corr), gk_ptr<int64_t>(d_gene_pos0), idx->d_del_bits, idx->d_lb_a, idx->d_lb_t,
                      idx->d_gene_pbase, idx->d_snp_ord};
   if (n_mates) {
-    GK_PROF(ctx, "tab_count", GK_KERNEL(tab_count, dim3(nblk(n_mates)), dim3(kThreads), 0, st, mates, n_mates, ix,
-                       nt, cnt, valid, d_err, ev_save, ev_more, lo_save, mask_save, mask_more));
+    if (mates)
+      GK_PROF(ctx, "tab_count", GK_KERNEL(tab_count<false>, dim3(nblk(n_mates)), dim3(kThreads), 0, st, mates, c_off, c_words, n_mates,
+                         ix, nt, cnt, valid, d_err, ev_save, ev_more, lo_save, mask_save, mask_more));
+    else
+      GK_PROF(ctx, "tab_count", GK_KERNEL(tab_count<true>, dim3(nblk(n_mates)), dim3(kThreads), 0, st, mates, c_off, c_words, n_mates,
+                         ix, nt, cnt, valid, d_err, ev_save, ev_more, lo_save, mask_save, mask_more));
   }
   int64_t* d_spill_pair = nullptr;
   uint32_t* wide_ev = nullptr;
@@ -1020,10 +1106,17 @@
                      d_spill_pair, n_spill, prefix, tab->d_novel_key));
 
   GK_HIP(gk_pool_malloc(ctx, (void**)&tab->d_ids, (size_t)(tab->n_ids + 1) * sizeof(uint32_t)));
+  gk_mate* expanded = nullptr;
   if (n_mates) {
     const bool two_walks = gk_test_hook("two_walks");
     if ((err & 4) || two_walks) {
-      GK_PROF(ctx, "tab_emit", GK_KERNEL(tab_emit, dim3(nblk(n_mates)), dim3(kThreads), 0, st, mates, n_mates, ix, nt,
+      const gk_mate* records = mates;
+      if (!records) {
+        GK_HIP(gk_pool_malloc(ctx, (void**)&expanded, (size_t)n_mates * sizeof(gk_mate)));
+        GK_KERNEL(mates_unpack_words, dim3(nblk(n_mates)), dim3(kThreads), 0, st, c_off, c_words, n_mates, expanded);
+        records = expanded;
+      }
+      GK_PROF(ctx, "tab_emit", GK_KERNEL(tab_emit, dim3(nblk(n_mates)), dim3(kThreads), 0, st, records, n_mates, ix, nt,
                          cnt, valid, tab->d_ids));
     } else {
       GK_PROF(ctx, "tab_expand", GK_KERNEL(tab_expand, dim3(nblk(n_mates, kExpandThreads)), dim3(kExpandThreads), 0, st, n_mates, idx->n_var,
@@ -1039,13 +1132,13 @@
   GK_HIP(gk_pool_malloc(ctx, (void**)&tab->d_off, (size_t)(4 * tab->n_valid + 1) * sizeof(uint32_t)));
   GK_HIP(gk_pool_malloc(ctx, (void**)&tab->d_pair_gene, (size_t)tab->n_valid + 1));
   GK_HIP(gk_pool_malloc(ctx, (void**)&tab->d_pair_nh, (size_t)tab->n_valid + 1));
-  GK_PROF(ctx, "gather_pairs", GK_KERNEL(gather_pairs, dim3(nblk(tab->n_valid + 1)), dim3(kThreads), 0, st, mates, tab->d_pair_src,
-                     tab->n_valid, cnt, tab->d_off, tab->d_pair_gene, tab->d_pair_nh, (uint32_t)tab->n_ids));
+  GK_PROF(ctx, "gather_pairs", GK_KERNEL(gather_pairs, dim3(nblk(tab->n_valid + 1)), dim3(kThreads), 0, st, mates, c_off, c_words,
+                     tab->d_pair_src, tab->n_valid, cnt, tab->d_off, tab->d_pair_gene, tab->d_pair_nh, (uint32_t)tab->n_ids));
   GK_HIP(hipGetLastError());
   GK_HIP(hipStreamSynchronize(st));
   gk_pool_free(ctx,cnt); gk_pool_free(ctx,valid); gk_pool_free(ctx,d_err); gk_pool_free(ctx,bitmap); gk_pool_free(ctx,prefix); gk_pool_free(ctx,wide_bits);
   gk_pool_free(ctx,ev_save); gk_pool_free(ctx,lo_save); gk_pool_free(ctx,mask_save); gk_pool_free(ctx,ev_more); gk_pool_free(ctx,mask_more);
-  gk_pool_free(ctx,d_spill_pair); gk_pool_free(ctx,wide_ev);
+  gk_pool_free(ctx,d_spill_pair); gk_pool_free(ctx,wide_ev); gk_pool_free(ctx,expanded);
   gk_pool_free(ctx,nt.keys); gk_pool_free(ctx,nt.seq); gk_pool_free(ctx,nt.rank);
   if (err & 2) {
     gk_set_error("a filter-passing mate carries more variant events than its record format allows (%d, wide %d)", kMaxEv,
diff --git a/kir_graph_amd/csrc/gk_typing.hip b/kir_graph_amd/csrc/gk_typing.hip
--- a/kir_graph_amd/csrc/gk_typing.hip
+++ b/kir_graph_amd/csrc/gk_typing.hip
@@ -84,6 +84,17 @@
     if (5 * q < p + q) f |= 2;
   }
   vflag[v] = f;
+}
+
+__global__ __launch_bounds__(kThreads) void mask_tallies(const uint32_t* __restrict__ full_pos,
+                                                         const uint32_t* __restrict__ full_neg,
+                                                         const uint8_t* __restrict__ vflag, int64_t n,
+                                                         uint32_t* __restrict__ cnt_pos, uint32_t* __restrict__ cnt_neg) {
+  const int64_t v = (int64_t)blockIdx.x * kThreads + threadIdx.x;
+  if (v >= n) return;
+  const uint8_t f = vflag[v];
+  cnt_pos[v] = (f & 1) ? 0u : full_pos[v];
+  cnt_neg[v] = (f & 2) ? 0u : full_neg[v];
 }
 
 __global__ __launch_bounds__(kThreads) void flag_nonempty(const int32_t* rows, int64_t n_rows, const uint32_t* off,
@@ -811,7 +822,8 @@
 }
 
 static int sample_prepare(gk_ctx* ctx, gk_tab* tab, int32_t multiple, gk_dptr d_vflag, gk_dptr d_cnt, gk_dptr d_rows,
-                          int64_t* gene_off_out, const Survivors* surv, bool keep_vflag = false, int rounds = 1);
+                          int64_t* gene_off_out, const Survivors* surv, bool keep_vflag = false, int rounds = 1,
+                          gk_dptr d_cnt_full = 0);
 
 int gk_sample_prepare(gk_ctx* ctx, gk_tab* tab, int32_t multiple, gk_dptr d_vflag, gk_dptr d_cnt, gk_dptr d_rows,
                       int64_t* gene_off_out) {
@@ -836,8 +848,18 @@
   return sample_prepare(ctx, tab, multiple, d_vflag, d_cnt, d_rows, gene_off_out, &s, true, 2);
 }
 
+int gk_sample_prepare_exon_from(gk_ctx* ctx, gk_tab* tab, int32_t multiple, gk_dptr d_vflag, gk_dptr d_cnt, gk_dptr d_rows,
+                                int64_t* gene_off_out, int64_t max_out, int32_t* ord_out, uint32_t* pos_out,
+                                uint32_t* neg_out, int64_t* n_out, gk_dptr d_cnt_full) {
+  GK_REQUIRE(ord_out && pos_out && neg_out && n_out && max_out >= 0, "null pointer");
+  GK_REQUIRE(d_cnt_full != d_cnt || !d_cnt, "the full model's tallies and the exon model's are two buffers");
+  Survivors s;
+  s.max_out = max_out; s.ord = ord_out; s.pos = pos_out; s.neg = neg_out; s.n_out = n_out; s.novel_key = nullptr;
+  return sample_prepare(ctx, tab, multiple, d_vflag, d_cnt, d_rows, gene_off_out, &s, true, 2, d_cnt_full);
+}
+
 static int sample_prepare(gk_ctx* ctx, gk_tab* tab, int32_t multiple, gk_dptr d_vflag, gk_dptr d_cnt, gk_dptr d_rows,
-                          int64_t* gene_off_out, const Survivors* surv, bool keep_vflag, int rounds) {
+                          int64_t* gene_off_out, const Survivors* surv, bool keep_vflag, int rounds, gk_dptr d_cnt_full) {
   gk_bind(ctx);
   GK_REQUIRE(ctx && tab && tab->idx && d_vflag && d_cnt && d_rows && gene_off_out, "null pointer");
   if (surv) *surv->n_out = 0;
@@ -898,11 +920,16 @@
   GK_HIP(hipMemsetAsync(maybe, 0, (size_t)tab->n_valid, st));
   for (int round = 0; round < rounds; ++round) {
     if (round) GK_HIP(hipMemsetAsync(cnt, 0, (size_t)(2 * nv) * sizeof(uint32_t), st));
-    GK_PROF(ctx, "count_ids_genes",
-            GK_KERNEL(count_ids_genes, dim3((unsigned)n_wg), dim3(kThreads), (size_t)max_local * 8 + kThreads * sizeof(uint32_t), st, part.d_rows,
-                      (const int32_t*)d_tab, (const int64_t*)(d_tab + o_row0), (const int64_t*)(d_tab + o_row1),
-                      tab->idx->d_gene_vbeg, max_local, tab->d_off, tab->d_ids, vflag, cnt, cnt + nv,
-                      round == rounds - 1 ? maybe : (uint8_t*)nullptr));
+    if (round == 0 && rounds > 1 && d_cnt_full) {
+      const uint32_t* full = gk_ptr<const uint32_t>(d_cnt_full);
+      GK_PROF(ctx, "mask_tallies", GK_KERNEL(mask_tallies, dim3(nblk(nv)), dim3(kThreads), 0, st, full, full + nv, vflag, nv, cnt, cnt + nv));
+    } else {
+      GK_PROF(ctx, "count_ids_genes",
+              GK_KERNEL(count_ids_genes, dim3((unsigned)n_wg), dim3(kThreads), (size_t)max_local * 8 + kThreads * sizeof(uint32_t), st, part.d_rows,
+                        (const int32_t*)d_tab, (const int64_t*)(d_tab + o_row0), (const int64_t*)(d_tab + o_row1),
+                        tab->idx->d_gene_vbeg, max_local, tab->d_off, tab->d_ids, vflag, cnt, cnt + nv,
+                        round == rounds - 1 ? maybe : (uint8_t*)nullptr));
+    }
     GK_PROF(ctx, "apply_correction", GK_KERNEL(apply_correction, dim3(nblk(nv)), dim3(kThreads), 0, st, cnt, cnt + nv, nv, vflag));
   }
   uint32_t *flag = nullptr, *kept = nullptr;
diff --git a/kir_graph_amd/engine.py b/kir_graph_amd/engine.py
--- a/kir_graph_amd/engine.py
+++ b/kir_graph_amd/engine.py
@@ -99,6 +99,7 @@
         else:
             self.mates = mates
         self.n_pairs = self.mates.size // 2
+        compact = getattr(self.mates, "words", None) if hasattr(self.mates, "records") else None
         h = C.c_void_p()
         d_table = d_pos0 = None
         if correction is not None:
@@ -106,10 +107,18 @@
             assert table.dtype == np.uint8 and table.shape == (int(pos0[-1]), 5) and len(pos0) == len(dindex.host.genes) + 1
             d_table = self.dev.put(np.ascontiguousarray(table).reshape(-1) if table.size else np.zeros(1, np.uint8))
             d_pos0 = self.dev.put(np.ascontiguousarray(pos0, dtype=np.int64))
+        wide = which = None
         if spill is not None and len(spill[1]):
             wide = np.ascontiguousarray(spill[0], dtype=_lib.MATE_WIDE_DTYPE)
             which = np.ascontiguousarray(spill[1], dtype=np.int64)
             assert len(wide) == 2 * len(which)
+        if compact is not None:
+            check(lib().gk_tabulate_compact(self.dev.ctx, dindex.handle, compact.ptr, self.n_pairs,
+                                            d_table.ptr if d_table else 0, d_pos0.ptr if d_pos0 else 0,
+                                            wide.ctypes.data if wide is not None else None,
+                                            which.ctypes.data if which is not None else None,
+                                            len(which) if which is not None else 0, C.byref(h)))
+        elif wide is not None:
             check(lib().gk_tabulate_spilled(self.dev.ctx, dindex.handle, self.mates.ptr, self.n_pairs,
                                             d_table.ptr if d_table else 0, d_pos0.ptr if d_pos0 else 0,
                                             wide.ctypes.data, which.ctypes.data, len(which), C.byref(h)))
@@ -128,7 +137,8 @@
             raise AssertionError("variant window has left > right (graphkir/hisat2.py:744)")
         self._novel_keys = None
         if self.dev.call_log is not None:
-            self.dev.call_log.append(("tab_count", self.n_pairs, self.n_valid, self.n_ids))
+            self.dev.call_log.append(("tab_count", self.n_pairs, self.n_valid, self.n_ids)
+                                     + ((compact.nbytes,) if compact is not None else ()))
 
     @property
     def n_var_total(self) -> int:
@@ -172,7 +182,11 @@
                 args = (dev.ctx, self.handle, int(multiple), vflag.ptr, cnt.ptr, rows.ptr, off.ctypes.data, nv,
                         o.ctypes.data, p.ctypes.data, q.ctypes.data, C.byref(n_surv))
                 if exon:
-                    check(lib().gk_sample_prepare_exon(*args))
+                    full = store.get(bool(multiple))
+                    if full is not None:
+                        check(lib().gk_sample_prepare_exon_from(*args, full.cnt.ptr))
+                    else:
+                        check(lib().gk_sample_prepare_exon(*args))
                 else:
                     want_novel = self._novel_keys is None and self.n_novel > 0
                     novel_keys = np.empty(self.n_novel, dtype=np.uint64) if want_novel else None
diff --git a/kir_graph_amd/hisat2.py b/kir_graph_amd/hisat2.py
--- a/kir_graph_amd/hisat2.py
+++ b/kir_graph_amd/hisat2.py
@@ -227,9 +227,15 @@
         self.n_pairs, self.novel_base = tab.n_pairs, tab.novel_base
         self.expect = (tab.n_valid, tab.n_ids, tab.n_novel)
         self.spill, self.correction = getattr(tab, "_spill", None), getattr(tab, "_correction", None)
-        ptr, nbytes = C.c_uint64(), C.c_int64()
-        check(lib().gk_mates_compact(self.dev.ctx, tab.mates.ptr, 2 * self.n_pairs, C.byref(ptr), C.byref(nbytes)))
-        self.ptr, self.nbytes = ptr.value, int(nbytes.value)
+        self._words = None
+        words = getattr(tab.mates, "words", None) if hasattr(tab.mates, "records") else None
+        if words is not None:
+            self._words, tab.mates.words = words, None
+            self.ptr, self.nbytes = words.ptr, int(words.nbytes)
+        else:
+            ptr, nbytes = C.c_uint64(), C.c_int64()
+            check(lib().gk_mates_compact(self.dev.ctx, tab.mates.ptr, 2 * self.n_pairs, C.byref(ptr), C.byref(nbytes)))
+            self.ptr, self.nbytes = ptr.value, int(nbytes.value)
         self.dev.sync()
         tab.mates.free()
         tab.mates = None
@@ -238,9 +244,14 @@
     def restore(self) -> "SampleData":
         if not self.ptr:
             raise ValueError("restored already")
-        mates = self.dev.alloc(2 * self.n_pairs, _lib.MATE_DTYPE)
-        check(lib().gk_mates_expand(self.dev.ctx, self.ptr, 2 * self.n_pairs, mates.ptr))
-        self.release()
+        if self._words is not None:
+            from .packed import DeviceCompactMates
+            mates = DeviceCompactMates(self._words.dev, self._words, 2 * self.n_pairs)
+            self._words, self.ptr = None, 0
+        else:
+            mates = self.dev.alloc(2 * self.n_pairs, _lib.MATE_DTYPE)
+            check(lib().gk_mates_expand(self.dev.ctx, self.ptr, 2 * self.n_pairs, mates.ptr))
+            self.release()
         tab = Tabulation(self.dindex, mates, novel_base=self.novel_base, dev=self.dev, spill=self.spill,
                          correction=self.correction)
         if (tab.n_valid, tab.n_ids, tab.n_novel) != self.expect:
@@ -249,7 +260,10 @@
         return SampleData(tab, self.index, None, ins_strings=self.ins_strings)
 
     def release(self) -> None:
-        if self.ptr:
+        if self._words is not None:
+            self._words.free()
+            self._words, self.ptr = None, 0
+        elif self.ptr:
             lib().gk_free(self.dev.ctx, self.ptr)
             self.ptr = 0
 
diff --git a/kir_graph_amd/packed.py b/kir_graph_amd/packed.py
--- a/kir_graph_amd/packed.py
+++ b/kir_graph_amd/packed.py
@@ -1,6 +1,7 @@
 from __future__ import annotations
 
 import re
+import threading
 
 import numpy as np
 
@@ -475,6 +476,50 @@
     return (before - before[first]).astype(np.int64)
 
 
+class DeviceCompactMates:
+
+    def __init__(self, dev, words, n_mates: int):
+        from ._lib import MATE_DTYPE
+        self.dev, self.words, self.n_mates = dev, words, int(n_mates)
+        self.dtype, self.shape = MATE_DTYPE, (self.n_mates,)
+        self._records = None
+        self._lock = threading.Lock()
+
+    @property
+    def size(self) -> int:
+        return self.n_mates
+
+    @property
+    def nbytes(self) -> int:
+        return int(self.words.nbytes if self.words is not None else 0) + int(self._records.nbytes if self._records is not None else 0)
+
+    def records(self):
+        with self._lock:
+            if self._records is None:
+                from ._lib import check, lib
+                if self.words is None:
+                    raise ValueError("the compact records have been released already")
+                records = self.dev.alloc(self.n_mates, self.dtype)
+                check(lib().gk_mates_expand(self.dev.ctx, self.words.ptr, self.n_mates, records.ptr))
+                self.dev.sync()
+                self._records = records
+            return self._records
+
+    @property
+    def ptr(self) -> int:
+        return self.records().ptr
+
+    def download(self, count: int | None = None, offset: int = 0) -> np.ndarray:
+        return self.records().download(count, offset)
+
+    def free(self) -> None:
+        with self._lock:
+            for b in (self.words, self._records):
+                if b is not None:
+                    b.free()
+            self.words = self._records = None
+
+
 class CompactMates:
 
     def __init__(self, records: np.ndarray, threads: int = 4):
@@ -492,14 +537,11 @@
     def nbytes(self) -> int:
         return int(self.words.nbytes)
 
-    def toDevice(self, dev, wait: bool = False):
+    def toDevice(self, dev, wait: bool = False) -> DeviceCompactMates:
         import ctypes as C
-        from ._lib import MATE_DTYPE, check, lib
-        compact = dev.alloc(len(self.words), np.uint32)
-        check(lib().gk_h2d_async(dev.ctx, compact.ptr, C.c_void_p(self.words.ctypes.data), self.words.nbytes))
-        mates = dev.alloc(self.n_mates, MATE_DTYPE)
-        check(lib().gk_mates_expand(dev.ctx, compact.ptr, self.n_mates, mates.ptr))
-        compact.free()
+        from ._lib import check, lib
+        words = dev.alloc(len(self.words), np.uint32)
+        check(lib().gk_h2d_async(dev.ctx, words.ptr, C.c_void_p(self.words.ctypes.data), self.words.nbytes))
         if wait:
             dev.sync()
-        return mates
+        return DeviceCompactMates(dev, words, self.n_mates)
diff --git a/kir_graph_amd/roofmodel.py b/kir_graph_amd/roofmodel.py
--- a/kir_graph_amd/roofmodel.py
+++ b/kir_graph_amd/roofmodel.py
@@ -46,8 +46,9 @@
     return 4.0 * n_ids + 16.0 * n_rows + float(out_bytes + 1) * n_rows * n_allele, 4.0 * n_ids * n_allele
 
 
-def tabLaunch(n_pairs: int, n_valid: int, n_ids: int) -> tuple[float, float]:
-    return 256.0 * n_pairs + 4.0 * n_ids + 22.0 * n_valid, 0.0
+def tabLaunch(n_pairs: int, n_valid: int, n_ids: int, record_bytes: float | None = None) -> tuple[float, float]:
+    read = 256.0 * n_pairs if record_bytes is None else float(record_bytes)
+    return read + 4.0 * n_ids + 22.0 * n_valid, 0.0
 
 
 def setsumLaunch(n_rows: int, n_sets: int, c: int, n_distinct: int) -> tuple[float, float]:
@@ -84,7 +85,7 @@
         elif kernel == "compat_rows8":
             b, o = compatLaunch(*c[1:5])[0], 0.0
         elif kernel == "tab_count":
-            b, o = tabLaunch(*c[1:4])
+            b, o = tabLaunch(*c[1:5])
         elif kernel in ("fraction_chunks", "setsum_leaves"):
             b, o = setsumLaunch(*c[1:5])
         else:
diff --git a/kir_graph_amd/samtools_utils.py b/kir_graph_amd/samtools_utils.py
--- a/kir_graph_amd/samtools_utils.py
+++ b/kir_graph_amd/samtools_utils.py
@@ -34,8 +34,13 @@
     off = np.zeros(len(genes) + 1, dtype=np.int64)
     np.cumsum(lens, out=off[1:])
     depth = np.empty(int(off[-1]), dtype=np.uint32)
-    check(lib().gk_depth(tab.dev.ctx, tab.handle, tab.mates.ptr, int(multiple), off.ctypes.data, len(genes),
-                         depth.ctypes.data))
+    words = getattr(tab.mates, "words", None) if hasattr(tab.mates, "records") else None
+    if words is not None:
+        check(lib().gk_depth_compact(tab.dev.ctx, tab.handle, words.ptr, int(multiple), off.ctypes.data, len(genes),
+                                     depth.ctypes.data))
+    else:
+        check(lib().gk_depth(tab.dev.ctx, tab.handle, tab.mates.ptr, int(multiple), off.ctypes.data, len(genes),
+                             depth.ctypes.data))
     if file_depth:
         names = (C.c_char_p * len(genes))(*[g.encode() for g in genes])
         check(lib().gk_depth_write_tsv(file_depth.encode(), names, off.ctypes.data, len(genes), depth.ctypes.data))
```

Measured after the change: 520.1 million, median of 6. 9.7% higher.
